# tmoroney/whisper-diarize-rs

Measured on AMD Instinct MI355X. Metric: audio-sec/wall-sec (xRT), large-v3 + DTW + diarize, 1/2/4/8 MI355X, higher is better.
Workload: dtype f16 (f32 accumulate)

## Files before the change

include/wdr.h:

```cpp
#ifndef WDR_H
#define WDR_H

#include <stddef.h>
#include <stdint.h>

#ifdef __cplusplus
extern "C" {
#endif

#define WDR_ABI_VERSION 6

typedef struct wdr_engine wdr_engine;
typedef struct wdr_context wdr_context;

typedef struct {
  const char* cache_dir;
  int8_t enable_dtw;
  int8_t enable_flash_attn;
  int8_t use_gpu;
  int8_t has_gpu_device;
  int32_t gpu_device;
  const char* vad_model_path;
  const char* diarize_segment_model_path;
  const char* diarize_embedding_model_path;
// ... 74 lines not shown
  double start, end;
  const int16_t* samples; size_t n_samples;
} wdr_speech_segment;

typedef struct {
  void* user;
  void (*progress)(void* user, int32_t pct, int32_t type , const char* label);
  void (*new_segment)(void* user, const wdr_segment* seg);
  int (*is_cancelled)(void* user);
} wdr_callbacks;

typedef struct {
  double mel, encode, decode, dtw, vad, total;
  int64_t windows, decode_steps, prefills;
  double lang, prompt_gpu, embed;
  int64_t chains, batch_launches, batch_rows, fixup_segments, replay_segments;
  double spec_s, fixup_s;
  double batch_step_s;
  int64_t early_fixup_segments;
  int64_t batch_prefill_rows, batch_dtw_rows, batch_prefills, batch_dtws, batch_mixed;
  int64_t batch_xattn_groups, batch_xattn_tiles;
  int64_t dtwq_passes, dtwq_rows, dtwq_jobs;
  int64_t lang_passes, lang_rows;
} wdr_stage_times;

const char* wdr_last_error(void);
int wdr_abi_version(void);
int wdr_device_count(void);
void wdr_shutdown(void);

int wdr_engine_new(const wdr_engine_config* cfg, wdr_engine** out);
void wdr_engine_free(wdr_engine* e);
int wdr_engine_set_synthetic(wdr_engine* e, const wdr_synthetic* syn);
int wdr_engine_set_audio_convert(wdr_engine* e, int8_t on);
int wdr_engine_set_channel_split(wdr_engine* e, int8_t on);
int wdr_transcribe_audio(wdr_engine* e, const char* audio_path, const wdr_transcribe_options* opts,
                         const wdr_formatting_overrides* fmt, const wdr_callbacks* cb, wdr_segment_list** out);

int wdr_read_wav(const char* path, int16_t** samples, size_t* n);
int wdr_audio_info(const char* path, int32_t* info, uint64_t* n_frames);
int wdr_read_audio(const char* path, int8_t has_gpu_device, int32_t gpu_device, int16_t** samples, size_t* n);
int wdr_read_audio_channels(const char* path, int8_t has_gpu_device, int32_t gpu_device,
                            int16_t** samples, size_t* n_per_channel, int32_t* channels);
int wdr_dbg_model_file(int32_t kind, const char* path, char** names_out, float** data_out, size_t* n_values);
int wdr_process_segments(const wdr_segment* segs, size_t n_segs, const char* lang, const wdr_formatting_overrides* ov,
                         int8_t has_mask, const double* vad_mask, size_t n_mask, wdr_segment_list** out);
void wdr_free(void* p);
int wdr_vad_merge(const double* starts_cs, const double* ends_cs, size_t n_segs, const int16_t* samples,
                  size_t n_samples, double* mask_out , size_t* n_mask,
                  double* merged_out , int64_t* merged_idx ,
                  size_t* n_merged);
typedef struct wdr_vad wdr_vad;
int wdr_vad_create(const char* model_path, int8_t has_gpu_device, int32_t gpu_device, wdr_vad** out);
void wdr_vad_free(wdr_vad* v);
int wdr_vad_probs(wdr_vad* v, const int16_t* samples, size_t n, float* probs_out, double* us_per_step);
int wdr_vad_stats(wdr_vad* v, double* us_per_chunk);
int wdr_vad_segments_from_probs(const float* probs, size_t n_probs, float* cs_out, size_t* n_out);
int wdr_vad_get_segments(wdr_vad* v, const int16_t* samples, size_t n, double** mask_out, size_t* n_mask,
                         wdr_speech_segment** segs_out, size_t* n_segs);

typedef struct wdr_diarizer wdr_diarizer;
int wdr_diarizer_create(const char* segment_model_path, const char* embedding_model_path, int8_t has_gpu_device,
                        int32_t gpu_device, wdr_diarizer** out);
void wdr_diarizer_free(wdr_diarizer* d);
int wdr_diarize_frame_classes(wdr_diarizer* d, const int16_t* samples, size_t n, int32_t* cls_out, float* logprobs_out);
int wdr_diarize_get_segments(wdr_diarizer* d, const int16_t* samples, size_t n, wdr_speech_segment** segs_out,
                             size_t* n_segs);
int wdr_diarize_segments_from_classes(const int32_t* cls, size_t n_windows, const int16_t* samples, size_t n,
                                      wdr_speech_segment** segs_out, size_t* n_segs);
int wdr_diarize_fbank(wdr_diarizer* d, const int16_t* samples, size_t n, float* feats_out, size_t* n_frames);
int wdr_diarize_embedding(wdr_diarizer* d, const int16_t* samples, size_t n, float* emb_out, int8_t* ok);
int wdr_diarize_embedding_batch(wdr_diarizer* d, const int16_t* const* samples, const size_t* n, int32_t B,
                                float* emb_out, int8_t* ok);
int wdr_diarize_stats(wdr_diarizer* d, double* seg_ms, double* emb_ms);
typedef struct wdr_speakers wdr_speakers;
int wdr_speakers_new(int8_t has_max_speakers, uint64_t max_speakers, wdr_speakers** out);
void wdr_speakers_free(wdr_speakers* m);
int wdr_speakers_assign(wdr_speakers* m, const float* emb, int32_t dim, float threshold, char* id_out, size_t cap);

int wdr_context_create(const char* model_path, const char* model_name, int8_t has_gpu_device, int32_t gpu_device,
                       int8_t use_gpu, int8_t enable_dtw, int8_t enable_flash_attn, int8_t has_num_samples,
                       uint64_t num_samples, const wdr_synthetic* syn, wdr_context** out);
void wdr_context_free(wdr_context* c);
int wdr_ggml_info(const char* path, int32_t* hparams, int64_t* n_tensors, int64_t* n_vocab_tokens);
int wdr_ggml_tensor_types(const char* path, int64_t* counts );
int wdr_ggml_tensor_f16(const char* path, const char* name, uint16_t** out, size_t* n);
int wdr_run_pipeline(wdr_context* c, const wdr_speech_segment* segs, size_t n_segs, const wdr_transcribe_options* opts,
                     const wdr_diarize_options* diarize, const wdr_synthetic* syn, const wdr_callbacks* cb,
                     wdr_segment_list** out);
int wdr_run_pipeline_raw(wdr_context* c, const wdr_speech_segment* segs, size_t n_segs,
                         const wdr_transcribe_options* opts, const wdr_synthetic* syn, wdr_segment_list** out);
int wdr_run_pipeline_block(wdr_context* c, const wdr_speech_segment* segs, size_t n_segs,
                           const wdr_transcribe_options* opts, const wdr_synthetic* syn, const char* rng_in,
                           int8_t* sampled_out, char** rng_out, wdr_segment_list** out);
void wdr_segment_list_free(wdr_segment_list* l);
int wdr_context_set_chains(wdr_context* c, int32_t n);
int wdr_context_devices(const wdr_context* c, int32_t* n, int32_t* device_ids, int32_t cap);
int wdr_context_set_encoder_fp8(wdr_context* c, int8_t on);
int wdr_dbg_set_early_fixup(wdr_context* c, int32_t mode);
int wdr_dbg_set_gemm32(int32_t mfma);
int wdr_context_stage_times(wdr_context* c, wdr_stage_times* out);
int wdr_context_hparams(wdr_context* c, int32_t* out );

int wdr_prof_set(int32_t cls);
int wdr_prof_set_mask(int32_t mask);
int wdr_prof_read_class(int32_t cls, double* total_ms, int64_t* launches, double* algo_bytes, double* algo_flops);
int wdr_prof_read_clock(int32_t cls, double* total_ms, int64_t* launches, double* algo_bytes, double* algo_flops);
int wdr_prof_read(double* total_ms, int64_t* launches, double* algo_bytes, double* algo_flops);

typedef struct {
  int32_t id, tid;
  float p, plog, pt, ptsum;
  int64_t t0, t1, t_dtw;
} wdr_token;
typedef struct {
  int64_t t0, t1;
  const char* text;
  const wdr_token* tokens; size_t n_tokens;
} wdr_result_seg;
int wdr_state_full(wdr_context* c, const float* samples, size_t n, const wdr_transcribe_options* opts,
                   const wdr_synthetic* syn, const char* initial_prompt, wdr_result_seg** segs, size_t* n_segs,
                   int32_t* lang_id);
void wdr_result_free(wdr_result_seg* segs, size_t n);

int wdr_dbg_log_mel(wdr_context* c, const float* x, size_t n, int32_t seek, float* window_out );
int wdr_dbg_energy(const float* x, size_t n, float* out);
int wdr_dbg_dequant(int32_t type, const uint8_t* blocks, size_t n_blocks, uint16_t* out_f16, double* ms);
int wdr_dbg_audio_convert(const uint8_t* raw, uint64_t n_frames, int32_t fmt, int32_t channels, int32_t rate,
                          uint64_t chunk_frames, int32_t host, int16_t** out, size_t* n_out, double* ms);
int wdr_dbg_audio_split(const uint8_t* raw, uint64_t n_frames, int32_t fmt, int32_t channels, int32_t rate,
                        uint64_t chunk_frames, int32_t host, int16_t** out, size_t* n_per_channel, double* ms);
int wdr_dbg_resample_table(int32_t rate, int32_t* L, int32_t* M, int32_t* T, float** tab);
int wdr_dbg_mfma_scale(const uint8_t* a, const uint8_t* b, const int32_t* sa, const int32_t* sb, float* out);
int wdr_dbg_encode(wdr_context* c, const float* mel_window , float* enc_out );
int wdr_dbg_cross_kv(wdr_context* c, float* out);
int wdr_dbg_decode(wdr_context* c, const int32_t* tokens, size_t n, float* logits_out );
int wdr_dbg_step(wdr_context* c, const int32_t* tokens, size_t n, float* logits_out );
int wdr_dbg_logits(wdr_context* c, const float* logits, int32_t R, const int32_t* ctl, const float* temperature,
                   float max_initial_ts, int32_t suppress_blank, int32_t* ids_out, float* f_out);
int wdr_dbg_batch_step(wdr_context* c, const int32_t* tokens, size_t n, int32_t rows, int32_t iters,
                       double* ms_per_step);
int wdr_dbg_capture(wdr_context* c, const int32_t* tokens, size_t n, float* cap_out );
int wdr_dbg_dtw(const float* cap, int32_t n_heads, int32_t n_tok, int32_t n_audio, int32_t sot_len, int32_t seek,
                float* x_out , int32_t* times_out, int32_t* n_times);
int wdr_dbg_discrete(const float* w, size_t n, uint32_t seed, int32_t n_draws, int32_t* out);
int wdr_dbg_dtw_dp(const float* x, int32_t rows, int32_t cols, int32_t seek, int32_t* times_out, int32_t* n_times);
int wdr_dbg_proj_fp8(const uint16_t* a_f16, const uint16_t* w_f16, const float* bias, int32_t M, int32_t N, int32_t K,
                     int32_t epi, float* out, uint8_t* a8_out, uint8_t* a_scale_out, uint8_t* w8_out,
                     uint8_t* w_scale_out);
int wdr_dbg_proj(const uint16_t* a_f16, const uint16_t* w_f16, const float* bias, int32_t M, int32_t N, int32_t K,
                 int32_t epi, float* out );
#define WDR_DBG_PROJ_ROWS 0x200
#define WDR_DBG_PROJ_GEMM1 0x800
int wdr_dbg_proj_ln(const float* x, const float* gamma, const float* beta, const uint16_t* w_f16, const float* bias,
                    int32_t M, int32_t N, int32_t K, int32_t epi, int32_t fused, float* out);
int wdr_dbg_attn(const uint16_t* q, const uint16_t* k, const uint16_t* v, int32_t Tq, int32_t Tk, int32_t n_head,
                 int32_t causal, float* out );
int wdr_dbg_xattn(const uint16_t* q, const uint16_t* kv, const int32_t* row_slot, const int32_t* grp, int32_t R,
                  int32_t S, int32_t H, int32_t iters, float* out);

int wdr_dbg_self_attn(const uint16_t* q, const uint16_t* kc, const uint16_t* vc, int32_t n_seq, int32_t T,
                      const int32_t* row_seq, const int32_t* row_pos, int32_t R, int32_t H, float* out);
int wdr_dbg_proj_qkv(const uint16_t* a_f16, const uint16_t* w_f16, const float* bias, int32_t M, int32_t d, int32_t K,
                     const int32_t* row_seq, const int32_t* row_pos, int32_t n_seq, int32_t T, uint16_t* kc_io,
                     uint16_t* vc_io, float* q_out);
int wdr_dbg_logits_topk(wdr_context* c, const float* logits, int32_t R, const int32_t* ctl, const float* temperature,
                        float max_initial_ts, int32_t suppress_blank, int32_t K, int32_t* ids_out, float* f_out);
int wdr_dbg_logits_probs(wdr_context* c, const float* logits, int32_t R, const int32_t* ctl, const float* temperature,
                         float max_initial_ts, int32_t suppress_blank, float* probs_out, float* logprobs_out);
int wdr_dbg_kv_rows(wdr_context* c, int32_t seq, int32_t n_rows, int32_t write, uint16_t* k, uint16_t* v);
int wdr_dbg_kv_reorder(wdr_context* c, const int32_t* src, const int32_t* dst, int32_t n, int32_t n_rows);

#ifdef __cplusplus
}
#endif
#endif
```

whisper-diarize-rs_amd/csrc/common.h:

```cpp
#pragma once

#include <hip/hip_runtime.h>
#include <hip/hip_fp16.h>

#include <cstdint>
#include <cstdio>
#include <stdexcept>
#include <string>

namespace wdr {

struct HipError : std::runtime_error {
  using std::runtime_error::runtime_error;
};

#define WDR_HIP(call)                                                                       \
  do {                                                                                      \
    hipError_t e_ = (call);                                                                 \
    if (e_ != hipSuccess)                                                                   \
      throw ::wdr::HipError(std::string("HIP error ") + hipGetErrorString(e_) + " at " +    \
                            __FILE__ + ":" + std::to_string(__LINE__) + " (" #call ")");    \
  } while (0)

#define WDR_CHECK(cond, msg)                                                                \
  do {                                                                                      \
    if (!(cond)) throw std::runtime_error(std::string(msg));                                \
  } while (0)

typedef _Float16 f16;
typedef _Float16 f16x8 __attribute__((ext_vector_type(8)));
typedef _Float16 f16x4 __attribute__((ext_vector_type(4)));
typedef float f32x16 __attribute__((ext_vector_type(16)));
typedef float f32x4 __attribute__((ext_vector_type(4)));

enum Epi : int {
  EPI_F16 = 0,
  EPI_F16_GELU = 1,
  EPI_F32_RESID = 2,
  EPI_F32 = 3,
  EPI_F32_GELU_POS = 4,
  EPI_QKV_CACHE = 5,
  EPI_XKV = 6,
  EPI_F8_GELU = 7
};

constexpr int XKV_T = 1500;
constexpr long long XKV_HS = (long long)XKV_T * 64;
__host__ __device__ inline long long xkv_k_off(int l, int H) { return (long long)(2 * l) * H * XKV_HS; }
__host__ __device__ inline long long xkv_v_off(int l, int H) { return (long long)(2 * l + 1) * H * XKV_HS; }

__host__ __device__ inline int cdiv(int a, int b) { return (a + b - 1) / b; }

__device__ __forceinline__ float gelu_tanh(float x) {
#pragma clang fp contract(off)
  const float c2 = 2.0f * 0.7978845608028654f;
  const float u2 = c2 * __builtin_fmaf(0.044715f * x, x * x, x);
  float g = x * __builtin_amdgcn_rcpf(1.0f + __builtin_amdgcn_exp2f(u2 * -1.4426950408889634f));
  asm("" : "+v"(g));
  return g;
}

__device__ __forceinline__ float wave_sum(float v) {
  for (int o = 32; o > 0; o >>= 1) v += __shfl_xor(v, o, 64);
  return v;
}
__device__ __forceinline__ float wave_max(float v) {
  for (int o = 32; o > 0; o >>= 1) v = fmaxf(v, __shfl_xor(v, o, 64));
  return v;
}
__device__ __forceinline__ void lds_barrier() { asm volatile("s_waitcnt lgkmcnt(0)\n\ts_barrier" ::: "memory"); }

__device__ __forceinline__ double wave_sum_d(double v) {
  for (int o = 32; o > 0; o >>= 1) v += __shfl_xor(v, o, 64);
  return v;
}

struct ProjArgs {
  const f16* A; int lda;
  const f16* B; int ldb;
  const float* bias;
  void* out; int ldo;
  const float* pos; int pos_rows;
  int M, N, K;
  int epi;
  const float* ln_x = nullptr; int ldln = 0; const float* ln_g = nullptr; const float* ln_b = nullptr;
  f16* kc = nullptr; f16* vc = nullptr; long long seq_stride = 0; const int* row_seq = nullptr;
  const int* row_pos = nullptr; int d = 0;
  unsigned long long* ts = nullptr;
  const uint8_t* A8 = nullptr; const uint8_t* B8 = nullptr;
  const uint32_t* a_sc = nullptr; const uint32_t* b_sc = nullptr; int ld_asc = 0, ld_bsc = 0;
  uint32_t* o_sc = nullptr; int ld_osc = 0;
  int tile_gm = 0;
  int gemm_ref = 0;
  int rows_mma = 0;
  const int* row_map = nullptr;
};

constexpr int PROF_CLK_LANES = 128;
struct ProfClock {
  unsigned long long* ts;
  __device__ __forceinline__ explicit ProfClock(unsigned long long* t) : ts(t) {
    if (ts && threadIdx.x == 0) atomicMin(ts + lane_of_block(), (unsigned long long)wall_clock64());
  }
  __device__ __forceinline__ ~ProfClock() {
    if (ts && threadIdx.x == ((blockDim.x - 1) & ~63u)) atomicMax(ts + PROF_CLK_LANES + lane_of_block(), (unsigned long long)wall_clock64());
  }
  __device__ __forceinline__ static int lane_of_block() {
    return (int)((blockIdx.x + blockIdx.y * 7u + blockIdx.z * 13u) % PROF_CLK_LANES);
  }
};
unsigned long long* prof_slot();
template <typename A>
inline unsigned long long* prof_attach(A&) { return nullptr; }
inline unsigned long long* prof_attach(ProjArgs& a) { return a.ts = prof_slot(); }
void launch_proj(const ProjArgs& a, hipStream_t s);
void gemm_knobs_reload();
void launch_proj_fp8(const ProjArgs& a, hipStream_t s);
void launch_quant_f8(const f16* x, int ldx, int rows, int K, uint8_t* y, int ldy, uint32_t* sc, int ld_sc,
                     hipStream_t s);
void launch_probe_mfma_scale(const void* a, const void* b, const int* sa, const int* sb, float* out, hipStream_t s);
void launch_layernorm_f8(const float* x, int ldx, const float* g, const float* b, uint8_t* y, int ldy, uint32_t* sc,
                         int ld_sc, int rows, int d, hipStream_t s);

}
```

whisper-diarize-rs_amd/csrc/engine.cpp:

```cpp
#include <algorithm>
#include <atomic>
#include <chrono>
#include <cmath>
#include <cstdio>
#include <cstdlib>
#include <cstring>
#include <fstream>
#include <map>
#include <memory>
#include <random>
#include <string>
#include <sys/stat.h>
#include <dirent.h>
#include <condition_variable>
#include <exception>
#include <mutex>
#include <set>
#include <pthread.h>
#include <thread>
#include <vector>

#include "../../include/wdr.h"
#include "audio_file.h"
#include "audio_gpu.h"
// ... 2233 lines not shown

int wdr_dbg_decode(wdr_context* c, const int32_t* tokens, size_t n, float* logits_out) {
  WDR_GUARD({
    WDR_USE(ctx, c);
    c->st->decode_logits(tokens, (int)n, logits_out);
    return 0;
  })
}

int wdr_dbg_step(wdr_context* c, const int32_t* tokens, size_t n, float* logits_out) {
  WDR_GUARD({
    WDR_USE(ctx, c);
    c->st->dbg_step(tokens, (int)n, logits_out);
    return 0;
  })
}

int wdr_dbg_logits(wdr_context* c, const float* logits, int32_t R, const int32_t* ctl, const float* temperature,
                   float max_initial_ts, int32_t suppress_blank, int32_t* ids_out, float* f_out) {
  WDR_GUARD({
    WDR_USE(ctx, c);
    WDR_CHECK(R >= 1 && R <= 8, "dbg_logits: 1..8 rows");
    std::vector<LogitsCtl> lc(R);
    for (int r = 0; r < R; ++r) {
      const int32_t* q = ctl + 7 * r;
      lc[r] = LogitsCtl{q[0], q[1], q[2], q[3], q[4], q[5], q[6], temperature[r]};
    }
    std::vector<TokenData> out(R);
    std::vector<float> nosp(R);
    c->st->dbg_logits(logits, R, lc.data(), max_initial_ts, suppress_blank != 0, out.data(), nosp.data());
    for (int r = 0; r < R; ++r) {
      ids_out[2 * r] = out[r].id;
      ids_out[2 * r + 1] = out[r].tid;
      float* f = f_out + 5 * r;
      f[0] = out[r].p;
      f[1] = out[r].plog;
      f[2] = out[r].pt;
      f[3] = out[r].ptsum;
      f[4] = nosp[r];
    }
    return 0;
  })
}

int wdr_dbg_batch_step(wdr_context* c, const int32_t* tokens, size_t n, int32_t rows, int32_t iters,
                       double* ms_per_step) {
  WDR_GUARD({
    WDR_USE(ctx, c);
    *ms_per_step = c->st->dbg_batch_step(tokens, (int)n, rows, iters);
    return 0;
  })
}

int wdr_dbg_capture(wdr_context* c, const int32_t* tokens, size_t n, float* cap_out) {
  WDR_GUARD({
    WDR_USE(ctx, c);
    if (c->ctx->aheads.empty()) return fail("context created without DTW");
    c->st->dtw_capture(tokens, (int)n, cap_out);
    return 0;
  })
}

int wdr_dbg_dtw(const float* cap, int32_t A, int32_t N, int32_t M, int32_t sot_len, int32_t seek, float* x_out,
                int32_t* times_out, int32_t* n_times) {
  WDR_GUARD({
    DevMem dcap((size_t)A * N * 1500 * 4), dn((size_t)A * N * M * 4), dx((size_t)N * M * 4), dt((N + 8) * 4);
    WDR_HIP(hipMemcpy(dcap.p, cap, dcap.bytes, hipMemcpyHostToDevice));
    launch_dtw(dcap.as<float>(), A, N, 1500, M, sot_len, seek, dn.as<float>(), dx.as<float>(), dt.as<int>(),
               dt.as<int>() + N + 4, nullptr);
    WDR_HIP(hipDeviceSynchronize());
    const int rows = N - sot_len - 1;
    WDR_HIP(hipMemcpy(x_out, dx.p, (size_t)rows * M * 4, hipMemcpyDeviceToHost));
    std::vector<int> t(N + 8);
    WDR_HIP(hipMemcpy(t.data(), dt.p, t.size() * 4, hipMemcpyDeviceToHost));
    *n_times = t[N + 4];
    for (int i = 0; i < *n_times; ++i) times_out[i] = t[i];
    return 0;
  })
}

int wdr_dbg_dtw_dp(const float* x, int32_t rows, int32_t cols, int32_t seek, int32_t* times_out, int32_t* n_times) {
  WDR_GUARD({
    DevMem dx((size_t)rows * cols * 4), dt((rows + 8) * 4);
    WDR_HIP(hipMemcpy(dx.p, x, dx.bytes, hipMemcpyHostToDevice));
    launch_dtw_dp_only(dx.as<float>(), rows, cols, seek, dt.as<int>(), dt.as<int>() + rows + 4, nullptr);
    std::vector<int> t(rows + 8);
    WDR_HIP(hipMemcpy(t.data(), dt.p, t.size() * 4, hipMemcpyDeviceToHost));
    *n_times = t[rows + 4];
    for (int i = 0; i < *n_times; ++i) times_out[i] = t[i];
    return 0;
  })
}

int wdr_dbg_proj_fp8(const uint16_t* a16, const uint16_t* w16, const float* bias, int32_t M, int32_t N, int32_t K,
                     int32_t epi, float* out, uint8_t* a8_out, uint8_t* a_sc_out, uint8_t* w8_out, uint8_t* w_sc_out) {
  WDR_GUARD({
    WDR_CHECK(M > 64 && N % 256 == 0 && K % 128 == 0, "dbg fp8 projection: M > 64, N % 256, K % 128");
    const int mp = (M + 255) / 256 * 256;
    DevMem da((size_t)M * K * 2), dw((size_t)N * K * 2), db(bias ? (size_t)N * 4 : 0), dout((size_t)M * N * 4);
    DevMem a8((size_t)M * K), w8((size_t)N * K), as((size_t)K / 128 * mp * 4), ws((size_t)K / 128 * N * 4);
    DevMem osc((size_t)N / 128 * mp * 4);
    WDR_HIP(hipMemcpy(da.p, a16, da.bytes, hipMemcpyHostToDevice));
    WDR_HIP(hipMemcpy(dw.p, w16, dw.bytes, hipMemcpyHostToDevice));
    if (bias) WDR_HIP(hipMemcpy(db.p, bias, db.bytes, hipMemcpyHostToDevice));
    launch_quant_f8(da.as<f16>(), K, M, K, a8.as<uint8_t>(), K, as.as<uint32_t>(), mp, nullptr);
    launch_quant_f8(dw.as<f16>(), K, N, K, w8.as<uint8_t>(), K, ws.as<uint32_t>(), N, nullptr);
    const bool f16out = epi == EPI_F16 || epi == EPI_F16_GELU;
    if (!f16out && epi != EPI_F8_GELU) WDR_HIP(hipMemcpy(dout.p, out, dout.bytes, hipMemcpyHostToDevice));
    ProjArgs p{nullptr, K, nullptr, K, bias ? db.as<float>() : nullptr, dout.p, N, nullptr, 0, M, N, K, epi};
    p.A8 = a8.as<uint8_t>();
    p.a_sc = as.as<uint32_t>();
    p.ld_asc = mp;
    p.B8 = w8.as<uint8_t>();
    p.b_sc = ws.as<uint32_t>();
    p.ld_bsc = N;
    p.o_sc = osc.as<uint32_t>();
    p.ld_osc = mp;
    launch_proj_fp8(p, nullptr);
    WDR_HIP(hipDeviceSynchronize());
    auto unscale = [](const DevMem& d, int rows, int ld, int K, uint8_t* dst) {
      std::vector<uint32_t> h(d.bytes / 4);
      WDR_HIP(hipMemcpy(h.data(), d.p, d.bytes, hipMemcpyDeviceToHost));
      for (int r = 0; r < rows; ++r)
        for (int b = 0; b < K / 32; ++b) dst[(size_t)r * (K / 32) + b] = (uint8_t)(h[(size_t)(b / 4) * ld + r] >> (8 * (b % 4)));
    };
    if (epi == EPI_F8_GELU) {
      std::vector<uint8_t> q((size_t)M * N), sc((size_t)M * (N / 32));
      WDR_HIP(hipMemcpy(q.data(), dout.p, q.size(), hipMemcpyDeviceToHost));
      unscale(osc, M, mp, N, sc.data());
      for (int r = 0; r < M; ++r)
        for (int c = 0; c < N; ++c) {
          const uint8_t v = q[(size_t)r * N + c];
          const int e = (v >> 3) & 15, mt = v & 7;
          float x = e ? std::ldexp(1.0f + mt / 8.0f, e - 7) : std::ldexp(mt / 8.0f, -6);
          if ((v & 0x7f) == 0x7f) x = NAN;
          x = (v & 0x80) ? -x : x;
          out[(size_t)r * N + c] = std::ldexp(x, (int)sc[(size_t)r * (N / 32) + c / 32] - 127);
        }
    } else if (f16out) {
      std::vector<f16> h((size_t)M * N);
      WDR_HIP(hipMemcpy(h.data(), dout.p, h.size() * 2, hipMemcpyDeviceToHost));
      for (size_t i = 0; i < h.size(); ++i) out[i] = (float)h[i];
    } else {
      WDR_HIP(hipMemcpy(out, dout.p, dout.bytes, hipMemcpyDeviceToHost));
    }
    if (a8_out) WDR_HIP(hipMemcpy(a8_out, a8.p, a8.bytes, hipMemcpyDeviceToHost));
    if (a_sc_out) unscale(as, M, mp, K, a_sc_out);
    if (w8_out) WDR_HIP(hipMemcpy(w8_out, w8.p, w8.bytes, hipMemcpyDeviceToHost));
    if (w_sc_out) unscale(ws, N, N, K, w_sc_out);
    return 0;
  })
}

int wdr_dbg_proj(const uint16_t* a16, const uint16_t* w16, const float* bias, int32_t M, int32_t N, int32_t K,
                 int32_t epi, float* out) {
  WDR_GUARD({
    DevMem da((size_t)M * K * 2), dw((size_t)N * K * 2), db(bias ? (size_t)N * 4 : 0), dout((size_t)M * N * 4);
    WDR_HIP(hipMemcpy(da.p, a16, da.bytes, hipMemcpyHostToDevice));
    WDR_HIP(hipMemcpy(dw.p, w16, dw.bytes, hipMemcpyHostToDevice));
    if (bias) WDR_HIP(hipMemcpy(db.p, bias, db.bytes, hipMemcpyHostToDevice));
    if (epi & 0x100) return fail("WDR_DBG_PROJ_STEP: the decode-step GEMV schedule was removed (the row kernel serves every row count)");
    const bool rows = (epi & 0x200) != 0;
    if (epi & 0x400) return fail("WDR_DBG_PROJ_SPLIT: the split-K residual projections were removed (k_skinny runs them whole)");
    const bool gemm_ref = (epi & 0x800) != 0;
    epi &= 0xff;
    const bool f16out = epi == EPI_F16 || epi == EPI_F16_GELU;
    std::vector<f16> h16;
    if (!f16out) WDR_HIP(hipMemcpy(dout.p, out, dout.bytes, hipMemcpyHostToDevice));
    ProjArgs a{da.as<f16>(), K, dw.as<f16>(), K, bias ? db.as<float>() : nullptr, dout.p, N, nullptr, 0, M, N, K, epi};
    a.rows_mma = rows ? 1 : 0;
    a.gemm_ref = gemm_ref ? 1 : 0;
    launch_proj(a, nullptr);
    WDR_HIP(hipDeviceSynchronize());
    if (f16out) {
      h16.resize((size_t)M * N);
      WDR_HIP(hipMemcpy(h16.data(), dout.p, h16.size() * 2, hipMemcpyDeviceToHost));
      for (size_t i = 0; i < h16.size(); ++i) out[i] = (float)h16[i];
    } else {
      WDR_HIP(hipMemcpy(out, dout.p, dout.bytes, hipMemcpyDeviceToHost));
    }
    return 0;
  })
}

int wdr_dbg_proj_ln(const float* x, const float* gamma, const float* beta, const uint16_t* w16, const float* bias,
                    int32_t M, int32_t N, int32_t K, int32_t epi, int32_t fused, float* out) {
  WDR_GUARD({
    if (M < 1 || N < 1 || K < 128 || K > 1280 || K % 128) return fail("dbg_proj_ln: M >= 1, K % 128 == 0, K <= 1280");
    if (epi != EPI_F16 && epi != EPI_F16_GELU && epi != EPI_F32) return fail("dbg_proj_ln: epi 0, 1 or 3");
    DevMem dx((size_t)M * K * 4), dg((size_t)K * 4), dbt((size_t)K * 4), dw((size_t)N * K * 2),
        db(bias ? (size_t)N * 4 : 0), dh((size_t)M * K * 2), dout((size_t)M * N * 4);
    WDR_HIP(hipMemcpy(dx.p, x, dx.bytes, hipMemcpyHostToDevice));
    WDR_HIP(hipMemcpy(dg.p, gamma, dg.bytes, hipMemcpyHostToDevice));
    WDR_HIP(hipMemcpy(dbt.p, beta, dbt.bytes, hipMemcpyHostToDevice));
    WDR_HIP(hipMemcpy(dw.p, w16, dw.bytes, hipMemcpyHostToDevice));
    if (bias) WDR_HIP(hipMemcpy(db.p, bias, db.bytes, hipMemcpyHostToDevice));
    ProjArgs a{nullptr, K, dw.as<f16>(), K, bias ? db.as<float>() : nullptr, dout.p, N, nullptr, 0, M, N, K, epi};
    a.rows_mma = 1;
    if (fused) {
      a.ln_x = dx.as<float>();
      a.ldln = K;
      a.ln_g = dg.as<float>();
      a.ln_b = dbt.as<float>();
    } else {
      launch_layernorm(dx.as<float>(), K, dg.as<float>(), dbt.as<float>(), dh.as<f16>(), K, M, K, nullptr);
      a.A = dh.as<f16>();
    }
    launch_proj(a, nullptr);
    WDR_HIP(hipDeviceSynchronize());
    if (epi == EPI_F32) {
      WDR_HIP(hipMemcpy(out, dout.p, dout.bytes, hipMemcpyDeviceToHost));
    } else {
      std::vector<f16> h((size_t)M * N);
      WDR_HIP(hipMemcpy(h.data(), dout.p, h.size() * 2, hipMemcpyDeviceToHost));
      for (size_t i = 0; i < h.size(); ++i) out[i] = (float)h[i];
    }
    return 0;
  })
}

int wdr_dbg_attn(const uint16_t* q, const uint16_t* k, const uint16_t* v, int32_t Tq, int32_t Tk, int32_t H,
                 int32_t causal, float* out) {
  WDR_GUARD({
    const int d = H * 64;
    DevMem dq((size_t)Tq * d * 2), dk((size_t)Tk * d * 2), dv((size_t)Tk * d * 2), dout((size_t)Tq * d * 2);
    WDR_HIP(hipMemcpy(dq.p, q, dq.bytes, hipMemcpyHostToDevice));
    WDR_HIP(hipMemcpy(dk.p, k, dk.bytes, hipMemcpyHostToDevice));
    WDR_HIP(hipMemcpy(dv.p, v, dv.bytes, hipMemcpyHostToDevice));
    FlashArgs fa{dq.as<f16>(), d, 0, dk.as<f16>(), d, 0, dv.as<f16>(), d, 0, dout.as<f16>(), d, 0, nullptr, Tq, Tk, H,
                 causal, 0.125f};
    DevMem po, pml;
    if (!causal && Tq <= 256 && Tk >= 512) {
      fa.nsplit = 12;
      po = DevMem((size_t)12 * Tq * H * 64 * 4);
      pml = DevMem((size_t)12 * H * Tq * 8);
      fa.part_o = po.as<float>();
      fa.part_ml = pml.as<float2>();
    }
    launch_flash_attn(fa, 1, nullptr);
    std::vector<f16> h((size_t)Tq * d);
    WDR_HIP(hipMemcpy(h.data(), dout.p, h.size() * 2, hipMemcpyDeviceToHost));
    for (size_t i = 0; i < h.size(); ++i) out[i] = (float)h[i];
    return 0;
  })
}

int wdr_dbg_xattn(const uint16_t* q, const uint16_t* kv, const int32_t* row_slot, const int32_t* grp, int32_t R,
                  int32_t S, int32_t H, int32_t iters, float* out) {
  WDR_GUARD({
    WDR_CHECK(R >= 1 && R <= 1024 && S >= 1 && H >= 1 && H <= 32 && iters >= 1, "dbg xattn: bad shape");
    const int d = H * 64, T = 1500;
    DevMem dq((size_t)R * d * 2), dkv((size_t)S * T * 2 * d * 2), dout((size_t)R * d * 2);
    DevMem po((size_t)24 * R * H * 64 * 4), pml((size_t)24 * R * H * 8);
    DevMem drk(R * sizeof(void*)), dg(R * 4), dl(R * 4);
    WDR_HIP(hipMemcpy(dq.p, q, dq.bytes, hipMemcpyHostToDevice));
    WDR_HIP(hipMemcpy(dkv.p, kv, dkv.bytes, hipMemcpyHostToDevice));
    XAttnArgs xa{dq.as<f16>(), d, dkv.as<f16>(), dkv.as<f16>() + d, 2 * d, T, R, H, 0.125f, po.as<float>(),
                 pml.as<float2>(), dout.as<f16>(), d};
    if (row_slot) {
      std::vector<const f16*> rk(R);
      for (int r = 0; r < R; ++r) {
        WDR_CHECK(row_slot[r] >= 0 && row_slot[r] < S, "dbg xattn: slot out of range");
        rk[r] = dkv.as<f16>() + (size_t)row_slot[r] * T * 2 * d;
      }
      WDR_HIP(hipMemcpy(drk.p, rk.data(), R * sizeof(void*), hipMemcpyHostToDevice));
      xa.row_k = drk.as<const f16*>();
      xa.v_off = d;
      bool big = false;
      for (int r = 0; grp && r < R; ++r) big = big || grp[r] > XATTN_GRP_MAX;
      if (grp && big) {
        std::vector<int> g(R, 0), lead;
        std::vector<int4> tiles;
        for (int r = 0; r < R; ++r) {
          if (grp[r] == 0) continue;
          WDR_CHECK(r + grp[r] <= R, "dbg xattn: bad group");
          if (grp[r] <= XATTN_GRP_MAX) {
            g[r] = grp[r];
            lead.push_back(r);
          } else {
            for (int t = 0; t < grp[r]; t += 128) tiles.push_back(make_int4(r + t, std::min(128, grp[r] - t), 1 << 30, 0));
          }
        }
        WDR_HIP(hipMemcpy(dg.p, g.data(), R * 4, hipMemcpyHostToDevice));
        if (!lead.empty()) WDR_HIP(hipMemcpy(dl.p, lead.data(), lead.size() * 4, hipMemcpyHostToDevice));
        DevMem dt(std::max<size_t>(16, tiles.size() * 16));
        if (!tiles.empty()) WDR_HIP(hipMemcpy(dt.p, tiles.data(), tiles.size() * 16, hipMemcpyHostToDevice));
        xa.grp = dg.as<int>();
        xa.lead = dl.as<int>();
        xa.n_vgrp = (int)lead.size();
        xa.vgrp_max = 1;
        for (int r : lead) xa.vgrp_max = std::max(xa.vgrp_max, g[r]);
        xa.tiles = dt.as<int4>();
        xa.n_tiles = (int)tiles.size();
        for (int i = 0; i < iters; ++i) launch_xattn_rows(xa, nullptr);
        WDR_HIP(hipDeviceSynchronize());
        std::vector<f16> h((size_t)R * d);
        WDR_HIP(hipMemcpy(h.data(), dout.p, h.size() * 2, hipMemcpyDeviceToHost));
        for (size_t i = 0; i < h.size(); ++i) out[i] = (float)h[i];
        return 0;
      }
      if (grp) {
        int ng = 0;
        for (int r = 0; r < R; ++r) {
          WDR_CHECK(grp[r] >= 0 && grp[r] <= XATTN_GRP_MAX && r + grp[r] <= R, "dbg xattn: bad group");
          ng += grp[r] > 0;
        }
        WDR_HIP(hipMemcpy(dg.p, grp, R * 4, hipMemcpyHostToDevice));
        xa.grp = dg.as<int>();
        xa.n_grp = ng;
        std::vector<int> lead;
        for (int r = 0; r < R; ++r)
          if (grp[r] > 0) lead.push_back(r);
        WDR_HIP(hipMemcpy(dl.p, lead.data(), lead.size() * 4, hipMemcpyHostToDevice));
        xa.lead = dl.as<int>();
      }
    }
    for (int i = 0; i < iters; ++i) launch_xattn(xa, nullptr);
    WDR_HIP(hipDeviceSynchronize());
    std::vector<f16> h((size_t)R * d);
    WDR_HIP(hipMemcpy(h.data(), dout.p, h.size() * 2, hipMemcpyDeviceToHost));
    for (size_t i = 0; i < h.size(); ++i) out[i] = (float)h[i];
    return 0;
  })
}

static void check_rows(const int32_t* row_seq, const int32_t* row_pos, int R, int n_seq, int T, const char* what) {
  for (int r = 0; r < R; ++r) {
    WDR_CHECK(row_seq[r] >= 0 && row_seq[r] < n_seq, std::string(what) + ": row_seq out of range");
    WDR_CHECK(row_pos[r] >= 0 && row_pos[r] < std::min(T, 448), std::string(what) + ": row_pos out of range");
  }
}

int wdr_dbg_self_attn(const uint16_t* q, const uint16_t* kc, const uint16_t* vc, int32_t n_seq, int32_t T,
                      const int32_t* row_seq, const int32_t* row_pos, int32_t R, int32_t H, float* out) {
  WDR_GUARD({
    WDR_CHECK(q && kc && vc && row_seq && row_pos && out, "dbg self-attn: null argument");
    WDR_CHECK(R >= 1 && R <= 4096 && H >= 1 && H <= 32 && n_seq >= 1 && n_seq <= 64 && T >= 1 && T <= 4096,
              "dbg self-attn: bad shape");
    check_rows(row_seq, row_pos, R, n_seq, T, "dbg self-attn");
    const int d = H * 64;
    const size_t cache = (size_t)n_seq * T * d * 2;
    DevMem dq((size_t)R * d * 2), dk(cache), dv(cache), dout((size_t)R * d * 2), ds(R * 4), dp(R * 4);
    WDR_HIP(hipMemcpy(dq.p, q, dq.bytes, hipMemcpyHostToDevice));
    WDR_HIP(hipMemcpy(dk.p, kc, cache, hipMemcpyHostToDevice));
    WDR_HIP(hipMemcpy(dv.p, vc, cache, hipMemcpyHostToDevice));
    WDR_HIP(hipMemcpy(ds.p, row_seq, R * 4, hipMemcpyHostToDevice));
    WDR_HIP(hipMemcpy(dp.p, row_pos, R * 4, hipMemcpyHostToDevice));
    DecSelfArgs sa{dq.as<f16>(), d, dk.as<f16>(), dv.as<f16>(), (long long)T * d, d, ds.as<int>(), dp.as<int>(),
                   dout.as<f16>(), d, 0.125f};
    launch_dec_self_attn(sa, R, H, nullptr);
    WDR_HIP(hipDeviceSynchronize());
    std::vector<f16> h((size_t)R * d);
    WDR_HIP(hipMemcpy(h.data(), dout.p, h.size() * 2, hipMemcpyDeviceToHost));
    for (size_t i = 0; i < h.size(); ++i) out[i] = (float)h[i];
    return 0;
  })
}

int wdr_dbg_proj_qkv(const uint16_t* a16, const uint16_t* w16, const float* bias, int32_t M, int32_t d, int32_t K,
                     const int32_t* row_seq, const int32_t* row_pos, int32_t n_seq, int32_t T, uint16_t* kc_io,
                     uint16_t* vc_io, float* q_out) {
  WDR_GUARD({
    WDR_CHECK(a16 && w16 && row_seq && row_pos && kc_io && vc_io && q_out, "dbg qkv projection: null argument");
    WDR_CHECK(M >= 1 && M <= 4096 && d >= 64 && d <= 2048 && d % 64 == 0 && d % 8 == 0 && K >= 32 && K <= 8192 &&
                  K % 32 == 0 && n_seq >= 1 && n_seq <= 64 && T >= 1 && T <= 4096,
              "dbg qkv projection: bad shape (d = 64 H, K % 32)");
    check_rows(row_seq, row_pos, M, n_seq, T, "dbg qkv projection");
    std::set<long long> seen;
    for (int r = 0; r < M; ++r)
      WDR_CHECK(seen.insert((long long)row_seq[r] * T + row_pos[r]).second, "dbg qkv projection: a cache row named twice");
    const int N = 3 * d;
    const size_t cache = (size_t)n_seq * T * d * 2;
    DevMem da((size_t)M * K * 2), dw((size_t)N * K * 2), db(bias ? (size_t)N * 4 : 0), dq((size_t)M * d * 2), dk(cache),
        dv(cache), ds(M * 4), dp(M * 4);
    WDR_HIP(hipMemcpy(da.p, a16, da.bytes, hipMemcpyHostToDevice));
    WDR_HIP(hipMemcpy(dw.p, w16, dw.bytes, hipMemcpyHostToDevice));
    if (bias) WDR_HIP(hipMemcpy(db.p, bias, db.bytes, hipMemcpyHostToDevice));
    WDR_HIP(hipMemcpy(dk.p, kc_io, cache, hipMemcpyHostToDevice));
    WDR_HIP(hipMemcpy(dv.p, vc_io, cache, hipMemcpyHostToDevice));
    WDR_HIP(hipMemcpy(ds.p, row_seq, M * 4, hipMemcpyHostToDevice));
    WDR_HIP(hipMemcpy(dp.p, row_pos, M * 4, hipMemcpyHostToDevice));
    ProjArgs a{da.as<f16>(), K, dw.as<f16>(), K, bias ? db.as<float>() : nullptr, dq.p, d, nullptr, 0, M, N, K,
               EPI_QKV_CACHE};
    a.rows_mma = 1;
    a.kc = dk.as<f16>();
    a.vc = dv.as<f16>();
    a.seq_stride = (long long)T * d;
    a.row_seq = ds.as<int>();
    a.row_pos = dp.as<int>();
    a.d = d;
    launch_proj(a, nullptr);
    WDR_HIP(hipDeviceSynchronize());
    std::vector<f16> h((size_t)M * d);
    WDR_HIP(hipMemcpy(h.data(), dq.p, h.size() * 2, hipMemcpyDeviceToHost));
    for (size_t i = 0; i < h.size(); ++i) q_out[i] = (float)h[i];
    WDR_HIP(hipMemcpy(kc_io, dk.p, cache, hipMemcpyDeviceToHost));
    WDR_HIP(hipMemcpy(vc_io, dv.p, cache, hipMemcpyDeviceToHost));
    return 0;
  })
}

static void dbg_ctls(const int32_t* ctl, const float* temperature, int R, std::vector<LogitsCtl>& lc) {
  lc.resize(R);
  for (int r = 0; r < R; ++r) {
    const int32_t* q = ctl + 7 * r;
    lc[r] = LogitsCtl{q[0], q[1], q[2], q[3], q[4], q[5], q[6], temperature[r]};
  }
}

int wdr_dbg_logits_topk(wdr_context* c, const float* logits, int32_t R, const int32_t* ctl, const float* temperature,
                        float max_initial_ts, int32_t suppress_blank, int32_t K, int32_t* ids_out, float* f_out) {
  WDR_GUARD({
    WDR_USE(ctx, c);
    WDR_CHECK(logits && ctl && temperature && ids_out && f_out, "dbg_logits_topk: null argument");
    WDR_CHECK(R >= 1 && R <= 8, "dbg_logits_topk: 1..8 rows");
    WDR_CHECK(K >= 1 && K <= BEAM_KMAX, "dbg_logits_topk: K out of range");
    std::vector<LogitsCtl> lc;
    dbg_ctls(ctl, temperature, R, lc);
    std::vector<BeamCand> bc((size_t)R * K);
    c->st->dbg_logits_topk(logits, R, lc.data(), max_initial_ts, suppress_blank != 0, K, bc.data());
    for (int i = 0; i < R * K; ++i) {
      ids_out[i] = bc[i].id;
      f_out[2 * i] = bc[i].p;
      f_out[2 * i + 1] = bc[i].plog;
    }
    return 0;
  })
}

int wdr_dbg_logits_probs(wdr_context* c, const float* logits, int32_t R, const int32_t* ctl, const float* temperature,
                         float max_initial_ts, int32_t suppress_blank, float* probs_out, float* logprobs_out) {
  WDR_GUARD({
    WDR_USE(ctx, c);
    WDR_CHECK(logits && ctl && temperature && probs_out && logprobs_out, "dbg_logits_probs: null argument");
    WDR_CHECK(R >= 1 && R <= 8, "dbg_logits_probs: 1..8 rows");
    std::vector<LogitsCtl> lc;
    dbg_ctls(ctl, temperature, R, lc);
    c->st->dbg_logits_probs(logits, R, lc.data(), max_initial_ts, suppress_blank != 0, probs_out, logprobs_out);
    return 0;
  })
}

int wdr_dbg_kv_rows(wdr_context* c, int32_t seq, int32_t n_rows, int32_t write, uint16_t* k, uint16_t* v) {
  WDR_GUARD({
    WDR_USE(ctx, c);
    WDR_CHECK(k && v, "dbg_kv_rows: null argument");
    c->st->dbg_kv_rows(seq, n_rows, write != 0, k, v);
    return 0;
  })
}

int wdr_dbg_kv_reorder(wdr_context* c, const int32_t* src, const int32_t* dst, int32_t n, int32_t n_rows) {
  WDR_GUARD({
    WDR_USE(ctx, c);
    WDR_CHECK(src && dst, "dbg_kv_reorder: null argument");
    c->st->dbg_kv_reorder(src, dst, n, n_rows);
    return 0;
  })
}

}
```

whisper-diarize-rs_amd/csrc/kernels/gemm.hip:

```cpp
#include "../common.h"
#include "../prof.h"

#include <algorithm>
#include <cstdlib>

namespace wdr {

typedef _Float16 f16x2 __attribute__((ext_vector_type(2)));

constexpr int GB_M = 128, GB_N = 128, GB_K = 32;
constexpr int GLDS = GB_K + 8;

template <int EPI>
__device__ __forceinline__ void epi_store(const ProjArgs& a, int row, int col, float v) {
  if (row >= a.M || col >= a.N) return;
  if (a.bias) v += a.bias[col];
  if constexpr (EPI == EPI_F16) {
    ((f16*)a.out)[(size_t)row * a.ldo + col] = (f16)v;
  } else if constexpr (EPI == EPI_F16_GELU) {
    ((f16*)a.out)[(size_t)row * a.ldo + col] = (f16)gelu_tanh(v);
  } else if constexpr (EPI == EPI_F32_RESID) {
    float* o = (float*)a.out + (size_t)row * a.ldo + col;
    *o = *o + v;
  } else if constexpr (EPI == EPI_F32) {
// ... 1111 lines not shown
      static bool attrn = [] {
        WDR_HIP(hipFuncSetAttribute((const void*)k_gemm8n<EPI>, hipFuncAttributeMaxDynamicSharedMemorySize, (int)G8N_LDS));
        return true;
      }();
      (void)attrn;
      const int ntn = (a.N / 128) * cdiv(a.M, G3_M);
      wdr_launch(PROF_GEMM, bytes, flops, k_gemm8n<EPI>, dim3(ntn), dim3(512), G8N_LDS, s, g);
      return;
    }
  }
  const int ntiles = (a.N / G3_N) * cdiv(a.M, G3_M);
  wdr_launch(PROF_GEMM, bytes, flops, k_gemm8<EPI>, dim3(ntiles), dim3(512), G8_LDS, s, g);
}

void launch_proj_fp8(const ProjArgs& a, hipStream_t s) {
  WDR_CHECK(a.A8 && a.B8 && a.a_sc && a.b_sc, "fp8 projection: operands / scales missing");
  WDR_CHECK(a.M > 64 && a.N % 128 == 0 && (a.epi != EPI_F8_GELU || a.N % G3_N == 0) && a.K % G8_BK == 0 &&
                a.lda % 16 == 0 && a.ldb % 16 == 0,
            "fp8 projection: M > 64, N % 128 == 0 (N % 256 for the GELU -> fp8 epilogue), K % 128 == 0, "
            "lda / ldb % 16 required");
  WDR_CHECK(a.ld_asc >= cdiv(a.M, G3_M) * G3_M && a.ld_bsc >= a.N && a.ld_asc % 4 == 0 && a.ld_bsc % 4 == 0,
            "fp8 projection: scale images need the rows rounded up to 256");
  WDR_CHECK(a.epi != EPI_F8_GELU || (a.o_sc && a.ld_osc >= cdiv(a.M, G3_M) * G3_M && a.ldo % 16 == 0),
            "fp8 projection: GELU -> fp8 epilogue needs an output scale image");
  switch (a.epi) {
    case EPI_F16: launch_epi8<EPI_F16>(a, s); break;
    case EPI_F16_GELU: launch_epi8<EPI_F16_GELU>(a, s); break;
    case EPI_F32_RESID: launch_epi8<EPI_F32_RESID>(a, s); break;
    case EPI_F32: launch_epi8<EPI_F32>(a, s); break;
    case EPI_F8_GELU: launch_epi8<EPI_F8_GELU>(a, s); break;
    default: throw std::runtime_error("fp8 projection: unsupported epilogue");
  }
  WDR_HIP(hipGetLastError());
}

__global__ __launch_bounds__(256) void k_quant_f8(const f16* x, int ldx, int rows, int K, uint8_t* y, int ldy,
                                                  uint32_t* sc, int ld_sc) {
  const int row = blockIdx.x * 4 + (threadIdx.x >> 6), lane = threadIdx.x & 63;
  if (row >= rows) return;
  const f16* xr = x + (size_t)row * ldx;
  for (int c0 = 0; c0 < K; c0 += 512) {
    const int c = c0 + lane * 8;
    const bool ok = c < K;
    f16x8 v = ok ? *(const f16x8*)(xr + c) : f16x8{};
    float am = 0.f;
#pragma unroll
    for (int e = 0; e < 8; ++e) am = fmaxf(am, fabsf((float)v[e]));
    am = fmaxf(am, __shfl_xor(am, 1, 64));
    am = fmaxf(am, __shfl_xor(am, 2, 64));
    const int e = f8_block_exp(am);
    const float inv = f8_pow2(-e);
    const uint32_t lo = f8_pack4((float)v[0] * inv, (float)v[1] * inv, (float)v[2] * inv, (float)v[3] * inv);
    const uint32_t hi = f8_pack4((float)v[4] * inv, (float)v[5] * inv, (float)v[6] * inv, (float)v[7] * inv);
    if (ok) *(uint2*)(y + (size_t)row * ldy + c) = make_uint2(lo, hi);
    const int b = e + 127, base = lane & ~15;
    const uint32_t w = (uint32_t)__shfl(b, base, 64) | (uint32_t)__shfl(b, base + 4, 64) << 8 |
                       (uint32_t)__shfl(b, base + 8, 64) << 16 | (uint32_t)__shfl(b, base + 12, 64) << 24;
    if ((lane & 15) == 0 && ok) sc[(size_t)(c >> 7) * ld_sc + row] = w;
  }
}

__global__ __launch_bounds__(64) void k_probe_mfma_scale(const i32x8* a, const i32x8* b, const int* sa, const int* sb,
                                                          f32x4* out) {
  const int l = threadIdx.x;
  out[l] = __builtin_amdgcn_mfma_scale_f32_16x16x128_f8f6f4(a[l], b[l], f32x4{0.f, 0.f, 0.f, 0.f}, 0, 0, 0, sa[l], 0,
                                                             sb[l]);
}
void launch_probe_mfma_scale(const void* a, const void* b, const int* sa, const int* sb, float* out, hipStream_t s) {
  WDR_KLAUNCH(k_probe_mfma_scale, dim3(1), dim3(64), 0, s, (const i32x8*)a, (const i32x8*)b, sa, sb, (f32x4*)out);
  WDR_HIP(hipGetLastError());
}

void launch_quant_f8(const f16* x, int ldx, int rows, int K, uint8_t* y, int ldy, uint32_t* sc, int ld_sc,
                     hipStream_t s) {
  WDR_CHECK(rows >= 1 && K % 128 == 0 && ldx % 8 == 0 && ldy % 16 == 0 && ld_sc >= rows,
            "fp8 quantisation: K % 128, ldx % 8, ldy % 16, scale rows");
  WDR_KLAUNCH(k_quant_f8, dim3(cdiv(rows, 4)), dim3(256), 0, s, x, ldx, rows, K, y, ldy, sc, ld_sc);
  WDR_HIP(hipGetLastError());
}

__global__ __launch_bounds__(256) void k_layernorm_f8(const float* x, int ldx, const float* g, const float* b,
                                                      uint8_t* y, int ldy, uint32_t* sc, int ld_sc, int rows, int d) {
  const int row = blockIdx.x * 4 + (threadIdx.x >> 6);
  const int lane = threadIdx.x & 63;
  if (row >= rows) return;
  const float* xr = x + (long long)row * ldx;
  float v[5][4];
  float s = 0.f;
#pragma unroll
  for (int j = 0; j < 5; ++j) {
    const int c = lane * 4 + j * 256;
    const bool ok = c < d;
    const int cc = ok ? c : 0;
    const float4 q = *(const float4*)(xr + cc);
    v[j][0] = ok ? q.x : 0.f; v[j][1] = ok ? q.y : 0.f; v[j][2] = ok ? q.z : 0.f; v[j][3] = ok ? q.w : 0.f;
    s += (v[j][0] + v[j][1]) + (v[j][2] + v[j][3]);
  }
  s = wave_sum(s);
  const float mean = s / d;
  float s2 = 0.f;
#pragma unroll
  for (int j = 0; j < 5; ++j)
    if (lane * 4 + j * 256 < d)
#pragma unroll
      for (int e = 0; e < 4; ++e) {
        const float t = v[j][e] - mean;
        s2 += t * t;
      }
  s2 = wave_sum(s2);
  const float scale = 1.0f / sqrtf(s2 / d + 1e-5f);
#pragma unroll
  for (int j = 0; j < 5; ++j) {
    const int c = lane * 4 + j * 256;
    if (j * 256 >= d) break;
    const bool ok = c < d;
    const int cc = ok ? c : 0;
    const float4 g4 = *(const float4*)(g + cc);
    const float4 b4 = *(const float4*)(b + cc);
    const float gg[4] = {g4.x, g4.y, g4.z, g4.w}, bb[4] = {b4.x, b4.y, b4.z, b4.w};
    float o[4], am = 0.f;
#pragma unroll
    for (int e = 0; e < 4; ++e) {
      o[e] = ok ? (v[j][e] - mean) * scale * gg[e] + bb[e] : 0.f;
      am = fmaxf(am, fabsf(o[e]));
    }
    am = fmaxf(am, __shfl_xor(am, 1, 64));
    am = fmaxf(am, __shfl_xor(am, 2, 64));
    am = fmaxf(am, __shfl_xor(am, 4, 64));
    const int e = f8_block_exp(am);
    const float inv = f8_pow2(-e);
    if (ok) *(uint32_t*)(y + (size_t)row * ldy + c) = f8_pack4(o[0] * inv, o[1] * inv, o[2] * inv, o[3] * inv);
    const int bb8 = e + 127, base = lane & 32;
    const uint32_t w = (uint32_t)__shfl(bb8, base, 64) | (uint32_t)__shfl(bb8, base + 8, 64) << 8 |
                       (uint32_t)__shfl(bb8, base + 16, 64) << 16 | (uint32_t)__shfl(bb8, base + 24, 64) << 24;
    if ((lane & 31) == 0 && ok) sc[(size_t)(c >> 7) * ld_sc + row] = w;
  }
}

void launch_layernorm_f8(const float* x, int ldx, const float* g, const float* b, uint8_t* y, int ldy, uint32_t* sc,
                         int ld_sc, int rows, int d, hipStream_t s) {
  WDR_CHECK(d % 128 == 0 && d <= 1280 && ldx % 4 == 0 && ldy % 16 == 0 && ld_sc >= rows,
            "fp8 layernorm: d % 128, d <= 1280");
  WDR_KLAUNCH(k_layernorm_f8, dim3(cdiv(rows, 4)), dim3(256), 0, s, x, ldx, g, b, y, ldy, sc, ld_sc, rows, d);
  WDR_HIP(hipGetLastError());
}

template <int EPI, int MT, int NT, int W>
constexpr uint32_t skinny_red_bytes() { return (uint32_t)W * MT * NT * 4 * 64 * 4; }
template <int EPI, int MT, int NT, int W>
static uint32_t skinny_ln_lds(int K) {
  return std::max((uint32_t)16 * MT * K * 2, skinny_red_bytes<EPI, MT, NT, W>());
}

template <int EPI, int MT, int NT, int W = 4, bool LN = false, int UU = 0>
__global__ __launch_bounds__(W * 64) void k_skinny(ProjArgs a) {
  ProfClock prof_clock_(a.ts);
  __shared__ float red_s[LN ? 1 : W * MT * NT * 4 * 64];
  extern __shared__ __attribute__((aligned(16))) f16 xln[];
  float* red = LN ? (float*)xln : red_s;
  const int lane = threadIdx.x & 63, wid = threadIdx.x >> 6;
  const int n0 = blockIdx.x * 16 * NT;
  const int m0 = blockIdx.y * 16 * MT;
  const int fr = lane & 15, fk = 8 * (lane >> 4);
  f32x4 acc[MT][NT];
#pragma unroll
  for (int i = 0; i < MT; ++i)
#pragma unroll
    for (int j = 0; j < NT; ++j) acc[i][j] = (f32x4){0.f, 0.f, 0.f, 0.f};
  const int lds_ld = a.K;
  if constexpr (LN) {
    const int d = a.K;
    const int live = min(16 * MT, a.M - m0);
    for (int rr = wid; rr < live; rr += W) {
      int row = m0 + rr;
      if (a.row_map) row = a.row_map[row];
      const float* xr = a.ln_x + (long long)row * a.ldln;
      float v[5][4];
      float sm = 0.f;
#pragma unroll
      for (int j = 0; j < 5; ++j) {
        const int c = lane * 4 + j * 256;
        const bool ok = c < d;
        const int cc = ok ? c : 0;
        const float4 q = *(const float4*)(xr + cc);
        v[j][0] = ok ? q.x : 0.f; v[j][1] = ok ? q.y : 0.f; v[j][2] = ok ? q.z : 0.f; v[j][3] = ok ? q.w : 0.f;
        sm += (v[j][0] + v[j][1]) + (v[j][2] + v[j][3]);
      }
      sm = wave_sum(sm);
      const float mean = sm / d;
      float s2 = 0.f;
#pragma unroll
      for (int j = 0; j < 5; ++j)
        if (lane * 4 + j * 256 < d)
#pragma unroll
          for (int e = 0; e < 4; ++e) {
            const float t = v[j][e] - mean;
            s2 += t * t;
          }
      s2 = wave_sum(s2);
      const float scale = 1.0f / sqrtf(s2 / d + 1e-5f);
#pragma unroll
      for (int j = 0; j < 5; ++j) {
        const int c = lane * 4 + j * 256;
        if (c >= d) continue;
        const float4 g4 = *(const float4*)(a.ln_g + c);
        const float4 b4 = *(const float4*)(a.ln_b + c);
        const float gg[4] = {g4.x, g4.y, g4.z, g4.w}, bb[4] = {b4.x, b4.y, b4.z, b4.w};
        f16x4 o;
#pragma unroll
        for (int e = 0; e < 4; ++e) o[e] = (f16)((v[j][e] - mean) * scale * gg[e] + bb[e]);
        *(f16x4*)(xln + rr * lds_ld + ((((c >> 3) ^ (rr & 15))) << 3) + (c & 7)) = o;
      }
    }
    __syncthreads();
  }
  const f16* arow[MT];
#pragma unroll
  for (int i = 0; i < MT; ++i) {
    int m = m0 + i * 16 + fr;
    m = m < a.M ? m : a.M - 1;
    if (!LN && a.row_map) m = a.row_map[m];
    arow[i] = LN ? xln + (i * 16 + fr) * lds_ld : a.A + (size_t)m * a.lda + fk;
  }
  const f16* brow[NT];
#pragma unroll
  for (int j = 0; j < NT; ++j) {
    int n = n0 + j * 16 + fr;
    n = n < a.N ? n : a.N - 1;
    brow[j] = a.B + (size_t)n * a.ldb + fk;
  }
  constexpr int U = UU > 0 ? UU : (MT + NT) <= 3 ? 8 : 4;
  for (int k0 = wid * 32; k0 < a.K; k0 += 32 * W * U) {
    f16x8 bf[U][NT], af[U][MT];
#pragma unroll
    for (int u = 0; u < U; ++u) {
      const int k = k0 + u * 32 * W;
      const bool ok = k < a.K;
      const int kk = ok ? k : 0;
#pragma unroll
      for (int j = 0; j < NT; ++j) {
        const f16x8 t = *(const f16x8*)(brow[j] + kk);
        bf[u][j] = ok ? t : (f16x8){};
      }
#pragma unroll
      for (int i = 0; i < MT; ++i) {
        const f16x8 t = LN ? *(const f16x8*)(arow[i] + ((((kk >> 3) | (lane >> 4)) ^ fr) << 3))
                           : *(const f16x8*)(arow[i] + kk);
        af[u][i] = ok ? t : (f16x8){};
      }
    }
#pragma unroll
    for (int u = 0; u < U; ++u)
#pragma unroll
      for (int i = 0; i < MT; ++i)
#pragma unroll
        for (int j = 0; j < NT; ++j)
          acc[i][j] = __builtin_amdgcn_mfma_f32_16x16x32_f16(af[u][i], bf[u][j], acc[i][j], 0, 0, 0);
  }
  if constexpr (LN) __syncthreads();
#pragma unroll
  for (int i = 0; i < MT; ++i)
#pragma unroll
    for (int j = 0; j < NT; ++j)
#pragma unroll
      for (int r = 0; r < 4; ++r) red[(((wid * MT + i) * NT + j) * 4 + r) * 64 + lane] = acc[i][j][r];
  __syncthreads();
  for (int e = threadIdx.x; e < MT * NT * 4 * 64; e += W * 64) {
    const int l = e & 63, r = (e >> 6) & 3, j = (e >> 8) % NT, i = (e >> 8) / NT;
    float v = 0.f;
#pragma unroll
    for (int w = 0; w < W; ++w) v += red[(((w * MT + i) * NT + j) * 4 + r) * 64 + l];
    const int row = m0 + i * 16 + (l >> 4) * 4 + r, col = n0 + j * 16 + (l & 15);
    epi_store<EPI>(a, row, col, v);
  }
}



struct GemmKnobs {
  bool gemm1, gemm3, gemm5, gemm5w;
  int gemm4, tile_gm, cus;
};
static int env_int(const char* name, int def) {
  const char* e = getenv(name);
  return e ? atoi(e) : def;
}
static GemmKnobs read_knobs() {
  GemmKnobs k;
  k.gemm1 = env_int("WDR_GEMM1", 0) != 0;
  k.gemm3 = env_int("WDR_GEMM3", 1) != 0 && !k.gemm1;
  k.gemm4 = env_int("WDR_GEMM4", -1);
  k.tile_gm = env_int("WDR_GEMM4_GM", 4);
  k.gemm5 = env_int("WDR_GEMM5", 0) != 0;
  k.gemm5w = env_int("WDR_GEMM5_WIDE", 1) != 0;
  k.cus = env_int("WDR_GEMM_CUS", 0) / 8 * 8;
  return k;
}
static GemmKnobs& knobs() {
  static GemmKnobs k = read_knobs();
  return k;
}
void gemm_knobs_reload() { knobs() = read_knobs(); }

template <int EPI>
static void launch_epi(const ProjArgs& a, hipStream_t s) {
  const int ob = (EPI == EPI_F32_RESID || EPI == EPI_F32 || EPI == EPI_F32_GELU_POS) ? 4 : 2;
  const double bytes = (double)a.N * a.K * 2 + (double)a.M * a.K * 2 + (double)a.M * a.N * ob;
  const double flops = 2.0 * a.M * a.N * a.K;
  WDR_CHECK(a.M > 64, "encoder GEMM: more than 64 rows (fewer go to the row kernel)");
  const GemmKnobs& kn = knobs();
  const bool ref = kn.gemm1 || a.gemm_ref;
  const bool vec4 = a.ldo % 4 == 0 && (a.epi != EPI_QKV_CACHE || a.d % 4 == 0);
  const bool wide5 = kn.gemm5w && a.N >= 4096 && a.N < 16384 && a.M >= 4096;
  if (a.N % 128 == 0 && a.K % G3_BK == 0 && a.M >= 4096 && !ref && vec4 && kn.gemm4 != 0 &&
      (wide5 || (a.N < 2048 && kn.gemm5 && (a.N / G3_N) * cdiv(a.M, G3_M) < 192))) {
    static bool attr5 = [] {
      WDR_HIP(hipFuncSetAttribute((const void*)k_gemm5<EPI>, hipFuncAttributeMaxDynamicSharedMemorySize, (int)G5_LDS));
      return true;
    }();
    (void)attr5;
    ProjArgs g = a;
    g.tile_gm = kn.tile_gm;
    const int ntiles5 = (a.N / 128) * cdiv(a.M, G3_M);
    dim3 grid(kn.cus > 0 && kn.cus < ntiles5 ? kn.cus : ntiles5);
    wdr_launch(PROF_GEMM, bytes, flops, k_gemm5<EPI>, grid, dim3(512), G5_LDS, s, g);
  } else if (a.N % G3_N == 0 && a.K % G3_BK == 0 && !ref && vec4 &&
             (kn.gemm4 == 1 ||
              (kn.gemm4 != 0 && (a.M >= 4096 || a.N >= 16384 || (a.N >= 4096 && a.M > 1024) ||
                                 (a.N >= 3072 && a.M >= 2560))))) {
    static bool attr4 = [] {
      WDR_HIP(hipFuncSetAttribute((const void*)k_gemm4<EPI>, hipFuncAttributeMaxDynamicSharedMemorySize, (int)G4_LDS));
      return true;
    }();
    (void)attr4;
    const int ntiles = (a.N / G3_N) * cdiv(a.M, G3_M);
    dim3 grid(kn.cus > 0 && kn.cus < ntiles ? kn.cus : ntiles);
    ProjArgs g = a;
    g.tile_gm = kn.tile_gm;
    wdr_launch(PROF_GEMM, bytes, flops, k_gemm4<EPI>, grid, dim3(512), G4_LDS, s, g);
  } else if ((a.N >= 5120 || a.M >= 9000) && a.M > 2048 && a.N % G3_N == 0 && a.K % G3_BK == 0 && kn.gemm3 && !ref) {
    static bool attr = [] {
      WDR_HIP(hipFuncSetAttribute((const void*)k_gemm3<EPI>, hipFuncAttributeMaxDynamicSharedMemorySize, (int)G3_LDS));
      return true;
    }();
    (void)attr;
    dim3 grid((a.N / G3_N) * cdiv(a.M, G3_M));
    wdr_launch(PROF_GEMM, bytes, flops, k_gemm3<EPI>, grid, dim3(512), G3_LDS, s, a);
  } else if (a.K % G2_BK == 0 && a.N <= 4096 && !ref && vec4) {
    dim3 grid((a.N / GB_N) * cdiv(a.M, GB_M));
    wdr_launch(PROF_GEMM, bytes, flops, k_gemm2<EPI>, grid, dim3(256), 0, s, a);
  } else {
    dim3 grid(a.N / GB_N, cdiv(a.M, GB_M));
    wdr_launch(PROF_GEMM, bytes, flops, k_gemm<EPI>, grid, dim3(256), 0, s, a);
  }
}

static bool rows_pair_tiles() {
  static const bool v = env_int("WDR_ROWS_PAIR", 1) != 0;
  return v;
}
static int rows_mt_max() {
  static const int v = std::max(2, std::min(5, env_int("WDR_ROWS_MT", 2)));
  return v;
}

template <int EPI>
static void launch_rows_epi(const ProjArgs& a, hipStream_t s) {
  const double bytes = (double)a.N * a.K * 2;
  const double flops = 2.0 * a.M * a.N * a.K;
  const int mt = cdiv(a.M, 16);
  const bool ln = a.ln_x != nullptr;
  const bool wide = a.N >= 4096;
  const int prof = PROF_GEMV;
  if (!wide) {
    if (a.K > 2048) {
      WDR_CHECK(!ln, "row projection: LN prologue needs K <= 1280");
      if (mt >= 4 && rows_pair_tiles()) {
        const int m2 = std::min(mt, rows_mt_max());
        const dim3 g2(cdiv(a.N, 16), cdiv(mt, m2));
        if (m2 >= 4) wdr_launch(prof, bytes, flops, k_skinny<EPI, 4, 1, 16, false, 2>, g2, dim3(1024), 0, s, a);
        else if (m2 == 3) wdr_launch(prof, bytes, flops, k_skinny<EPI, 3, 1, 16, false, 5>, g2, dim3(1024), 0, s, a);
        else wdr_launch(prof, bytes, flops, k_skinny<EPI, 2, 1, 16, false, 5>, g2, dim3(1024), 0, s, a);
        return;
      }
      wdr_launch(prof, bytes, flops, k_skinny<EPI, 1, 1, 16, false, 12>, dim3(cdiv(a.N, 16), mt), dim3(1024), 0, s, a);
      return;
    }
    if (!ln && mt > 2 && rows_pair_tiles()) {
      const int m2 = std::min(mt, rows_mt_max());
      const dim3 g2(cdiv(a.N, 16), cdiv(mt, m2));
      if (m2 >= 5) wdr_launch(prof, bytes, flops, k_skinny<EPI, 5, 1, 8>, g2, dim3(512), 0, s, a);
      else if (m2 == 4) wdr_launch(prof, bytes, flops, k_skinny<EPI, 4, 1, 8>, g2, dim3(512), 0, s, a);
      else if (m2 == 3) wdr_launch(prof, bytes, flops, k_skinny<EPI, 3, 1, 8>, g2, dim3(512), 0, s, a);
      else wdr_launch(prof, bytes, flops, k_skinny<EPI, 2, 1, 8>, g2, dim3(512), 0, s, a);
      return;
    }
    dim3 grid(cdiv(a.N, 16), mt), blk(512);
    if (ln) wdr_launch(prof, bytes, flops, k_skinny<EPI, 1, 1, 8, true>, grid, blk, skinny_ln_lds<EPI, 1, 1, 8>(a.K), s, a);
    else wdr_launch(prof, bytes, flops, k_skinny<EPI, 1, 1, 8>, grid, blk, 0, s, a);
    return;
  }
  const int mtw = std::min(mt, ln ? 2 : 4);
  dim3 grid(cdiv(a.N, 32), cdiv(mt, mtw)), blk(512);
#define WDR_RW(MTV)                                                                                        \
  if (ln) wdr_launch(prof, bytes, flops, k_skinny<EPI, MTV, 2, 8, true>, grid, blk, skinny_ln_lds<EPI, MTV, 2, 8>(a.K), s, a); \
  else wdr_launch(prof, bytes, flops, k_skinny<EPI, MTV, 2, 8>, grid, blk, 0, s, a);
  if (mtw == 1) { WDR_RW(1) }
  else if (mtw == 2) { WDR_RW(2) }
  else if (mtw == 3) { WDR_RW(3) }
  else { WDR_RW(4) }
#undef WDR_RW
}

static void launch_rows(const ProjArgs& a, hipStream_t s) {
  WDR_CHECK(a.K % 32 == 0 && a.lda % 8 == 0 && a.ldb % 8 == 0, "row projection: K % 32, lda / ldb % 8");
  WDR_CHECK(!a.ln_x || (a.K <= 1280 && a.K % 128 == 0), "row projection LN prologue: K <= 1280, K % 128 == 0");
  WDR_CHECK(a.epi != EPI_QKV_CACHE || (a.kc && a.vc && a.row_seq && a.row_pos && a.d > 0), "qkv-cache epilogue args");
  switch (a.epi) {
    case EPI_F16: launch_rows_epi<EPI_F16>(a, s); break;
    case EPI_F16_GELU: launch_rows_epi<EPI_F16_GELU>(a, s); break;
    case EPI_F32_RESID: launch_rows_epi<EPI_F32_RESID>(a, s); break;
    case EPI_F32: launch_rows_epi<EPI_F32>(a, s); break;
    case EPI_QKV_CACHE: launch_rows_epi<EPI_QKV_CACHE>(a, s); break;
    default: throw std::runtime_error("row projection: bad epilogue");
  }
  WDR_HIP(hipGetLastError());
}

void launch_proj(const ProjArgs& a, hipStream_t s) {
  WDR_CHECK(a.M > 0 && a.K > 0 && a.N > 0, "projection: empty shape");
  if (a.rows_mma || a.M <= 64) {
    launch_rows(a, s);
    return;
  }
  WDR_CHECK(a.K % 8 == 0 && a.lda % 8 == 0 && a.ldb % 8 == 0, "projection: K/lda/ldb must be multiples of 8");
  WDR_CHECK(a.N % GB_N == 0, "gemm: N must be a multiple of 128");
  WDR_CHECK(a.K % GB_K == 0, "gemm: K must be a multiple of 32");
  WDR_CHECK(a.epi != EPI_QKV_CACHE || (a.kc && a.vc && a.row_seq && a.row_pos && a.d > 0), "qkv-cache epilogue args");
  switch (a.epi) {
    case EPI_F16: launch_epi<EPI_F16>(a, s); break;
    case EPI_F16_GELU: launch_epi<EPI_F16_GELU>(a, s); break;
    case EPI_F32_RESID: launch_epi<EPI_F32_RESID>(a, s); break;
    case EPI_F32: launch_epi<EPI_F32>(a, s); break;
    case EPI_F32_GELU_POS: launch_epi<EPI_F32_GELU_POS>(a, s); break;
    case EPI_QKV_CACHE: launch_epi<EPI_QKV_CACHE>(a, s); break;
    case EPI_XKV:
      WDR_CHECK(a.M > 64 && a.seq_stride > 0, "cross-K/V epilogue: encoder GEMM rows and a slot stride");
      launch_epi<EPI_XKV>(a, s);
      break;
    default: throw std::runtime_error("projection: bad epilogue");
  }
  WDR_HIP(hipGetLastError());
}

}
```

whisper-diarize-rs_amd/csrc/rows.cpp:

```cpp
#include "rows.h"
#include "prof.h"

#include <algorithm>
#include <cstdlib>
#include <cstring>

namespace wdr {

namespace {
constexpr int kTileRows = 128;
constexpr int kNoEnd = 1 << 30;
size_t up16(size_t x) { return (x + 15) & ~size_t(15); }
}

RowBatch::RowBatch(int cr, int cl, int cc) : cap_rows(cr), cap_logits(cl), cap_caps(cc) {
  std::lock_guard<std::recursive_mutex> g(hip_alloc_mutex());
  bytes_ = up16((size_t)cr * 4) * 5 + up16((size_t)cr * 4) + up16((size_t)cl * 4) + 2 * up16((size_t)cc * 4) +
           up16((size_t)(cr / 8 + 2 + cr / kTileRows + 2) * 16) + up16((size_t)cr * 8) + up16((size_t)cc * 8) + 256;
  WDR_HIP(hipHostMalloc((void**)&h_, bytes_, hipHostMallocDefault));
  d_ = DevMem(bytes_);
  WDR_HIP(hipEventCreateWithFlags(&ev_, hipEventDisableTiming));
}

RowBatch::~RowBatch() {
  std::lock_guard<std::recursive_mutex> g(hip_alloc_mutex());
  if (pending_) (void)hipEventSynchronize(ev_);
  if (ev_) (void)hipEventDestroy(ev_);
  if (h_) (void)hipHostFree(h_);
}

void RowBatch::clear() {
  if (pending_) {
    WDR_HIP(hipEventSynchronize(ev_));
    pending_ = false;
  }
  R = n_logit = n_vgrp = vgrp_max = n_tiles = n_cap = 0;
  tok_.clear(); pos_.clear(); seq_.clear(); grp_.clear(); lend_.clear(); lead_.clear(); lrow_.clear();
  crow_.clear(); cstride_.clear(); tiles_.clear(); xkv_.clear(); cdst_.clear();
}

int RowBatch::add(const RowGroupDesc& g) {
  WDR_CHECK(g.n >= 1 && g.xkv && g.tok, "row batch: empty group");
  WDR_CHECK(R + g.n <= cap_rows, "row batch: rows over capacity");
  const int r0 = R;
  for (int i = 0; i < g.n; ++i) {
    tok_.push_back(g.tok[i]);
    pos_.push_back(g.pos ? g.pos[i] : g.pos0 + i);
    seq_.push_back(g.seq ? g.seq[i] : g.seq0);
    xkv_.push_back(g.xkv);
    grp_.push_back(0);
    lend_.push_back(kNoEnd);
  }
  R += g.n;
  if (g.n <= XATTN_GRP_MAX) {
    grp_[r0] = g.n;
    lend_[r0] = g.l_end;
    lead_.push_back(r0);
    n_vgrp++;
    vgrp_max = std::max(vgrp_max, g.n);
  } else {
    for (int t = 0; t < g.n; t += kTileRows) tiles_.push_back(make_int4(r0 + t, std::min(kTileRows, g.n - t), g.l_end, 0));
    n_tiles = (int)tiles_.size();
  }
  int first_logit = -1;
  if (g.logits) {
    first_logit = n_logit;
    for (int i = g.logits == 1 ? g.n - 1 : 0; i < g.n; ++i) lrow_.push_back(r0 + i);
    n_logit = (int)lrow_.size();
    WDR_CHECK(n_logit <= cap_logits, "row batch: logit rows over capacity");
  }
  if (g.cap) {
    for (int i = 0; i < g.n; ++i) {
      crow_.push_back(r0 + i);
      cdst_.push_back(g.cap + (size_t)i * XKV_T);
      cstride_.push_back(g.n * XKV_T);
    }
    n_cap = (int)crow_.size();
    WDR_CHECK(n_cap <= cap_caps, "row batch: capture rows over capacity");
  }
  return first_logit;
}

void RowBatch::upload(RowsIO& io, hipStream_t s, bool copy, bool track) {
  WDR_CHECK(R >= 1, "row batch: no rows");
  if (io.seq_stride > 0 && io.layer_stride > 0) {
    const long long nseq = io.layer_stride / io.seq_stride;
    for (int i = 0; i < R; ++i) WDR_CHECK(seq_[i] >= 0 && seq_[i] < nseq, "row batch: KV sequence outside the pool");
  }
  size_t off = 0;
  auto put = [&](const void* src, size_t n) -> const void* {
    const size_t o = off;
    if (n) memcpy(h_ + o, src, n);
    off = up16(off + n);
    WDR_CHECK(off <= bytes_, "row batch: tables over capacity");
    return (const void*)(d_.as<char>() + o);
  };
  io.tok = (const int*)put(tok_.data(), (size_t)R * 4);
  io.pos = (const int*)put(pos_.data(), (size_t)R * 4);
  io.seq = (const int*)put(seq_.data(), (size_t)R * 4);
  io.grp = (const int*)put(grp_.data(), (size_t)R * 4);
  io.lend = (const int*)put(lend_.data(), (size_t)R * 4);
  io.lead = (const int*)put(lead_.data(), lead_.size() * 4);
  io.lrow = (const int*)put(lrow_.data(), lrow_.size() * 4);
  io.crow = (const int*)put(crow_.data(), crow_.size() * 4);
  io.cstride = (const int*)put(cstride_.data(), cstride_.size() * 4);
  io.tiles = (const int4*)put(tiles_.data(), tiles_.size() * 16);
  io.xkv = (const f16* const*)put(xkv_.data(), (size_t)R * sizeof(void*));
  io.cdst = (float* const*)put(cdst_.data(), cdst_.size() * sizeof(void*));
  io.n_vgrp = n_vgrp;
  io.vgrp_max = std::max(1, vgrp_max);
  io.n_tiles = n_tiles;
  io.n_logit = n_logit;
  io.n_cap = n_cap;
  if (!copy) return;
  WDR_HIP(wdr_memcpy_async(d_.p, h_, off, hipMemcpyHostToDevice, s));
  if (track) {
    WDR_HIP(hipEventRecord(ev_, s));
    pending_ = true;
  }
}

void RowsBufs::alloc(int r, int lr, int d, int H, int V) {
  std::lock_guard<std::recursive_mutex> g(hip_alloc_mutex());
  rows = r;
  logit_rows = lr;
  xd = DevMem((size_t)r * d * 4);
  hd = DevMem((size_t)r * d * 2);
  qkvd = DevMem((size_t)r * 3 * d * 2);
  attd = DevMem((size_t)r * d * 2);
  qx = DevMem((size_t)r * d * 2);
  mlpd = DevMem((size_t)r * 4 * d * 2);
  part_o = DevMem((size_t)24 * r * H * 64 * 4);
  part_ml = DevMem((size_t)24 * r * H * sizeof(float2));
  ml = DevMem((size_t)r * H * sizeof(float2));
  logits = DevMem((size_t)std::max(1, lr) * V * 4);
}

RowsIO RowsBufs::io(const Context& ctx, int V) const {
  RowsIO o{};
  o.xd = xd.as<float>();
  o.hd = hd.as<f16>();
  o.qkvd = qkvd.as<f16>();
  o.attd = attd.as<f16>();
  o.qx = qx.as<f16>();
  o.mlpd = mlpd.as<f16>();
  o.part_o = part_o.as<float>();
  o.part_ml = part_ml.as<float2>();
  o.ml = ml.as<float2>();
  o.logits = logits.as<float>();
  o.ldlogits = V;
  o.kc = ctx.kv_k.as<f16>();
  o.vc = ctx.kv_v.as<f16>();
  o.layer_stride = ctx.kv_layer_stride;
  o.seq_stride = ctx.kv_seq_stride;
  return o;
}

void rows_forward(const Context& ctx, const RowsIO& io, int R, hipStream_t s, int l_stop) {
  const Model& md = ctx.model;
  const HParams& hp = md.hp;
  const int d = hp.n_text_state, L = hp.n_text_layer, H = hp.n_text_head;
  const float scale = 1.0f / 8.0f;
  WDR_CHECK(R >= 1 && io.tok && io.xkv, "rows forward: no rows / tables");
  static const int ln_env = getenv("WDR_ROWS_LN_FUSE") ? atoi(getenv("WDR_ROWS_LN_FUSE")) : -1;
  const int fuse_qkv = ln_env >= 0 ? ln_env : 48, fuse_xq = ln_env >= 0 ? ln_env : 64,
            fuse_fc1 = ln_env >= 0 ? ln_env : 24, fuse_logits = ln_env >= 0 ? ln_env : 0;
  auto P = [&](const f16* A, int lda, const f16* W, const float* b, void* out, int ldo, int N, int K, int epi,
               const float* lng = nullptr, const float* lnb = nullptr, int fuse_max = 0) {
    ProjArgs a{A, lda, W, K, b, out, ldo, nullptr, 0, R, N, K, epi};
    a.rows_mma = 1;
    if (lng) {
      if (R <= fuse_max) {
        a.ln_x = io.xd;
        a.ldln = d;
        a.ln_g = lng;
        a.ln_b = lnb;
      } else {
        launch_layernorm(io.xd, d, lng, lnb, io.hd, d, R, d, s);
        a.A = io.hd;
        a.lda = d;
      }
    }
    return a;
  };
  launch_embed(md.tok_emb, md.dec_pos, io.tok, io.pos, R, d, io.xd, s);
  const bool any_cap = io.n_cap > 0 && ctx.aheads_per_layer.size() == (size_t)L;
  int cap_slot0 = 0;
  for (int l = 0; l < L; ++l) {
    const DecLayer& e = md.dec[l];
    f16* kc = io.kc + (size_t)l * io.layer_stride;
    f16* vc = io.vc + (size_t)l * io.layer_stride;
    ProjArgs q = P(nullptr, d, e.w_qkv, e.b_qkv, io.qkvd, 3 * d, 3 * d, d, EPI_QKV_CACHE, e.ln1_g, e.ln1_b, fuse_qkv);
    q.kc = kc;
    q.vc = vc;
    q.seq_stride = io.seq_stride;
    q.row_seq = io.seq;
    q.row_pos = io.pos;
    q.d = d;
    launch_proj(q, s);
    DecSelfArgs sa{io.qkvd, 3 * d, kc, vc, io.seq_stride, d, io.seq, io.pos, io.attd, d, scale};
    launch_dec_self_attn(sa, R, H, s);
    launch_proj(P(io.attd, d, e.w_o, e.b_o, io.xd, d, d, d, EPI_F32_RESID), s);
    launch_proj(P(nullptr, d, e.w_xq, e.b_xq, io.qx, d, d, d, EPI_F16, e.ln2_g, e.ln2_b, fuse_xq), s);
    XAttnArgs xa{io.qx, d, nullptr, nullptr, 64, XKV_T, R, H, scale, io.part_o, io.part_ml, io.attd, d};
    xa.row_k = io.xkv;
    xa.layer_off = xkv_k_off(l, H);
    xa.v_off = xkv_v_off(l, H) - xkv_k_off(l, H);
    xa.hs = XKV_HS;
    xa.grp = io.grp;
    xa.lead = io.lead;
    xa.n_grp = io.n_vgrp;
    xa.n_vgrp = io.n_vgrp;
    xa.vgrp_max = io.vgrp_max;
    xa.lend = io.lend;
    xa.layer = l;
    xa.tiles = io.tiles;
    xa.n_tiles = io.n_tiles;
    const bool cap_layer = any_cap && !ctx.aheads_per_layer[l].empty();
    xa.ml_out = cap_layer ? io.ml : nullptr;
    launch_xattn_rows(xa, s);
    if (cap_layer) {
      CaptureRowsArgs ca{io.qx, d, io.xkv, xkv_k_off(l, H), XKV_HS, io.ml,
                         ctx.aheads_dev.as<int>() + ctx.aheads_dev_off[l], io.crow, io.cdst, io.cstride,
                         io.n_cap, cap_slot0, XKV_T, H, scale};
      launch_aheads_capture_rows(ca, (int)ctx.aheads_per_layer[l].size(), s);
    }
    if (ctx.aheads_per_layer.size() == (size_t)L) cap_slot0 += (int)ctx.aheads_per_layer[l].size();
    if (l + 1 >= l_stop) return;
    launch_proj(P(io.attd, d, e.w_xo, e.b_xo, io.xd, d, d, d, EPI_F32_RESID), s);
    launch_proj(P(nullptr, d, e.w_fc1, e.b_fc1, io.mlpd, 4 * d, 4 * d, d, EPI_F16_GELU, e.ln3_g, e.ln3_b, fuse_fc1), s);
    launch_proj(P(io.mlpd, 4 * d, e.w_fc2, e.b_fc2, io.xd, d, d, 4 * d, EPI_F32_RESID), s);
  }
  if (io.n_logit > 0) {
    ProjArgs a{nullptr, d, md.tok_emb, d, nullptr, io.logits, io.ldlogits, nullptr, 0, io.n_logit, hp.n_vocab, d, EPI_F32};
    a.rows_mma = 1;
    if (io.n_logit <= fuse_logits) {
      a.ln_x = io.xd;
      a.ldln = d;
      a.ln_g = md.ln_g;
      a.ln_b = md.ln_b;
      a.row_map = io.lrow;
    } else {
      launch_layernorm_rows(io.xd, d, md.ln_g, md.ln_b, io.hd, d, io.n_logit, d, io.lrow, s);
      a.A = io.hd;
    }
    launch_proj(a, s);
  }
}

void dtw_rows_forward(const Context& ctx, const RowsIO& io, int R, int l_end, hipStream_t s) {
  WDR_CHECK(io.n_cap == R && ctx.aheads_per_layer.size() == (size_t)ctx.model.hp.n_text_layer,
            "DTW rows forward: every row a capture row, alignment heads known");
  WDR_CHECK(l_end >= 1 && l_end <= ctx.model.hp.n_text_layer, "DTW rows forward: bad last layer");
  rows_forward(ctx, io, R, s, l_end);
}

}
```

whisper-diarize-rs_amd/csrc/whisper.h:

```cpp
#pragma once

#include <exception>
#include <atomic>
#include <memory>
#include <mutex>
#include <string>
#include <utility>
#include <vector>

#include "common.h"
#include "kernels/kernels.h"
#include "vocab.h"

namespace wdr {

uint64_t fnv1a64(const std::string& s);

struct HParams {
  int n_vocab = 51864, n_audio_ctx = 1500, n_audio_state = 512, n_audio_head = 8, n_audio_layer = 6;
  int n_text_ctx = 448, n_text_state = 512, n_text_head = 8, n_text_layer = 6, n_mels = 80;
};
bool hparams_for(const std::string& name, HParams* hp);

std::vector<std::pair<int, int>> alignment_heads_for(const std::string& model_name);

std::recursive_mutex& hip_alloc_mutex();
hipStream_t dedicated_stream(const char* knob, bool def, int prio);
void destroy_stream_pools();

struct DevMem {
  void* p = nullptr;
  size_t bytes = 0;
  DevMem() = default;
  explicit DevMem(size_t n);
  ~DevMem();
  DevMem(const DevMem&) = delete;
  DevMem& operator=(const DevMem&) = delete;
  DevMem(DevMem&& o) noexcept : p(o.p), bytes(o.bytes) { o.p = nullptr; o.bytes = 0; }
  DevMem& operator=(DevMem&& o) noexcept;
  template <typename T> T* as() const { return (T*)p; }
};

struct EncLayer {
  f16 *w_qkv, *w_o, *w_fc1, *w_fc2;
  float *b_qkv, *b_o, *b_fc1, *b_fc2, *ln1_g, *ln1_b, *ln2_g, *ln2_b;
};
struct DecLayer {
  f16 *w_qkv, *w_o, *w_xq, *w_xo, *w_fc1, *w_fc2;
  float *b_qkv, *b_o, *b_xq, *b_xo, *b_fc1, *b_fc2;
  float *ln1_g, *ln1_b, *ln2_g, *ln2_b, *ln3_g, *ln3_b;
};

struct Model {
  HParams hp;
  int kp1 = 0;
  f16 *conv1_w = nullptr, *conv2_w = nullptr;
  float *conv1_b = nullptr, *conv2_b = nullptr, *enc_pos = nullptr, *ln_post_g = nullptr, *ln_post_b = nullptr;
  std::vector<EncLayer> enc;
  std::vector<DecLayer> dec;
  f16* w_xkv = nullptr;
  float* b_xkv = nullptr;
  f16* tok_emb = nullptr;
  float *dec_pos = nullptr, *ln_g = nullptr, *ln_b = nullptr;
  float *mel_filters = nullptr, *hann = nullptr, *cos_tab = nullptr, *sin_tab = nullptr;
  DevMem storage;
  size_t weight_bytes = 0;
};

std::vector<uint8_t> fp8_plan_for(int n_layer);

struct ContextParams {
  bool use_gpu = true;
  int gpu_device = 0;
  bool dtw = true;
  bool flash_attn = false;
  double weight_std = 0.02;
  double emb_std = 0.02;
};

class Context {
 public:
  Context(const std::string& model_name, const HParams& hp, const ContextParams& cp,
          const class GgmlFile* gf = nullptr);
  ~Context();
  std::string name;
  ContextParams cp;
  Model model;
  Vocab vocab;
  std::vector<std::pair<int, int>> aheads;
  std::vector<std::vector<int>> aheads_per_layer;
  DevMem aheads_dev;
  std::vector<int> aheads_dev_off;
  hipStream_t stream = nullptr;
  hipStream_t low_prime = nullptr;
  std::vector<hipStream_t> prime_streams;
  int max_chains = 1;
  DevMem kv_k, kv_v;
  long long kv_seq_stride = 0, kv_layer_stride = 0;
  std::vector<std::unique_ptr<class StepBatcher>> batchers;
  int n_batchers = 1;
  StepBatcher& step_batcher(int chain = 0);
  std::unique_ptr<class StepBatcher> prefill_b;
  bool prefill_split = false;
  StepBatcher& prefill_batcher();
  std::unique_ptr<class DtwQueue> dtwq;
  class DtwQueue& dtw_queue();
  struct BatchStats {
    long long launches = 0, rows = 0, prefill_rows = 0, dtw_rows = 0, prefills = 0, dtws = 0, mixed = 0;
    long long vgroups = 0, tiles = 0;
    double step_s = 0;
    long long dq_passes = 0, dq_rows = 0, dq_jobs = 0;
  };
  BatchStats batcher_stats();
  std::atomic<bool> fp8_encoder{false};
  std::vector<uint8_t> fp8_plan;
  enum { F8_QKV = 1, F8_O = 2, F8_FC1 = 4, F8_FC2 = 8 };
  struct Fp8W {
    DevMem w, s;
  };
  struct Fp8Layer {
    Fp8W qkv, o, fc1, fc2;
  };
  const std::vector<Fp8Layer>& fp8_layers();

 private:
  std::mutex fp8_mu_;
  std::vector<Fp8Layer> fp8_layers_;
  void fp8_build();
};

struct FullParams {
  bool greedy = false;
  int best_of = 5, beam_size = 5;
  std::string language = "auto";
  bool translate = false;
  int n_max_text_ctx = 16384;
  std::string initial_prompt;
  bool has_initial_prompt = false;
  float temperature = 0.f, temperature_inc = 0.2f;
  float entropy_thold = 2.4f, logprob_thold = -1.f, no_speech_thold = 0.6f;
  float thold_pt = 0.01f, thold_ptsum = 0.01f, max_initial_ts = 1.f, length_penalty = -1.f;
  bool suppress_blank = true, single_segment = true, token_timestamps = true;
  int max_tokens = 0;
  float force_len_rate = 0.f;
};

struct TokenData {
  int id = 0, tid = 0;
  float p = 0, plog = 0, pt = 0, ptsum = 0;
  long long t0 = -1, t1 = -1, t_dtw = -1;
  float vlen = 0;
};

struct ResultSeg {
  long long t0, t1;
  std::string text;
  std::vector<TokenData> tokens;
};

struct StageTimes {
  double mel = 0, encode = 0, decode = 0, dtw = 0, glue = 0;
  long long windows = 0, decode_steps = 0, prefills = 0;
  double lang = 0, prompt_gpu = 0;
  long long lang_passes = 0, lang_rows = 0;
};

class StepBatcher {
 public:
  explicit StepBatcher(Context& ctx);
  ~StepBatcher();
  static constexpr int kRows = 8;
  struct Req {
    int n = 1;
    int tok[kRows], seq[kRows], pos[kRows];
    LogitsCtl ctl[kRows];
    const f16* xkv = nullptr;
    VocabIds vids{};
    int K = 0;
    TokenData out[kRows];
    BeamCand cand[kRows * BEAM_KMAX];
    int pn = 0;
    const int* ptok = nullptr;
    int pseq = 0;
    const f16* pxkv = nullptr;
    LogitsCtl pctl{};
    TokenData pout;
    float pnosp = 0.f;
    BeamCand pcand[BEAM_KMAX];
    int dn = 0;
    const int* dtok = nullptr;
    int dseq = 0;
    const f16* dxkv = nullptr;
    float* dcap = nullptr;
    int dl_end = 1 << 30;
    int ln = 0;
    int lseq = 0;
    const f16* lxkv = nullptr;
    float lout[100];
    bool done = false;
    std::exception_ptr err;
  };
  void enter();
  void leave();
  void step(Req& r);
  void run(std::vector<Req*>& batch) { launch(batch); }
  long long launches = 0, rows = 0, prefill_rows = 0, dtw_rows = 0, prefills = 0, dtws = 0, mixed = 0;
  long long vgroups = 0, tiles = 0;
  double step_s = 0;
  struct Impl;

 private:
  Context& ctx_;
  std::unique_ptr<Impl> m_;
  void launch(std::vector<Req*>& batch);
};
// ... 121 lines not shown
```

whisper-diarize-rs_amd/csrc/whisper_ctx.cpp:

```cpp
#include "whisper.h"
#include "rows.h"
#include "ggml_file.h"
#include "prof.h"

#include <algorithm>
#include <functional>
#include <chrono>
#include <cmath>
#include <cstring>
#include <cstdlib>
#include <map>
#include <random>
#include <exception>
#include <condition_variable>
#include <deque>
#include <set>
#include <pthread.h>
#include <thread>
#include <mutex>
#include <sstream>

namespace wdr {

static double now_s() {
// ... 362 lines not shown
  m.weight_bytes = A.off;
  m.storage = DevMem(A.off);
  char* base = m.storage.as<char>();
  auto h16 = [&](size_t o) { return (f16*)(base + o); };
  auto f32 = [&](size_t o) { return (float*)(base + o); };
  m.conv1_w = h16(o_c1w); m.conv1_b = f32(o_c1b); m.conv2_w = h16(o_c2w); m.conv2_b = f32(o_c2b);
  m.enc_pos = f32(o_epos); m.ln_post_g = f32(o_lnpg); m.ln_post_b = f32(o_lnpb);
  for (auto& e : eo)
    m.enc.push_back({h16(e.qkv), h16(e.o), h16(e.f1), h16(e.f2), f32(e.bqkv), f32(e.bo), f32(e.bf1), f32(e.bf2),
                     f32(e.l1g), f32(e.l1b), f32(e.l2g), f32(e.l2b)});
  for (auto& e : dd)
    m.dec.push_back({h16(e.qkv), h16(e.o), h16(e.xq), h16(e.xo), h16(e.f1), h16(e.f2), f32(e.bqkv), f32(e.bo),
                     f32(e.bxq), f32(e.bxo), f32(e.bf1), f32(e.bf2), f32(e.l1g), f32(e.l1b), f32(e.l2g), f32(e.l2b),
                     f32(e.l3g), f32(e.l3b)});
  m.w_xkv = h16(o_xkv); m.b_xkv = f32(o_bxkv); m.tok_emb = h16(o_tok); m.dec_pos = f32(o_dpos);
  m.ln_g = f32(o_lng); m.ln_b = f32(o_lnb);
  m.mel_filters = f32(o_filt); m.hann = f32(o_hann); m.cos_tab = f32(o_cos); m.sin_tab = f32(o_sin);

  hipStream_t s = stream;
  const double sq3 = std::sqrt(3.0);
  DevMem qstage;
  if (gf) {
    size_t mx = 0;
    for (const auto& kv : gf->tensors)
      if (kv.second.quantized()) mx = std::max(mx, kv.second.n_bytes());
    if (mx) qstage = DevMem((mx + 3) & ~size_t(3));
  }
  auto fill = [&](void* dst, const std::string& nm, long long rows, int src_cols, int dst_cols, bool is16, double sd) {
    if (!gf) {
      launch_synth_fill(dst, rows, src_cols, dst_cols, fnv1a64(nm), (float)(sd * sq3), is16, 0, 0.f, s);
      return;
    }
    const int64_t n = rows * (int64_t)src_cols;
    if (is16 && gf->get(nm).quantized()) {
      const GgmlTensor& t = gf->get(nm);
      WDR_CHECK(t.n_elem() == n, "failed to open model: tensor '" + nm + "' has " + std::to_string(t.n_elem()) +
                                     " elements, expected " + std::to_string(n));
      WDR_CHECK(dst_cols == src_cols, "ggml load: padded quantized tensor '" + nm + "'");
      WDR_CHECK(t.n_bytes() <= qstage.bytes, "ggml load: quantized staging buffer too small");
      WDR_HIP(hipMemcpy(qstage.p, t.data, t.n_bytes(), hipMemcpyHostToDevice));
      launch_dequant(t.type, qstage.p, n / 32, (f16*)dst, s);
      WDR_HIP(hipStreamSynchronize(s));
      return;
    }
    if (is16) {
      std::vector<uint16_t> v = gf->as_f16(nm, n), padded;
      if (dst_cols != src_cols) {
        padded.assign((size_t)rows * dst_cols, 0);
        for (long long r = 0; r < rows; ++r) memcpy(&padded[r * dst_cols], &v[r * src_cols], (size_t)src_cols * 2);
        v.swap(padded);
      }
      WDR_HIP(hipMemcpy(dst, v.data(), v.size() * 2, hipMemcpyHostToDevice));
    } else {
      WDR_CHECK(dst_cols == src_cols, "ggml load: padded f32 tensor");
      const std::vector<float> v = gf->as_f32(nm, n);
      WDR_HIP(hipMemcpy(dst, v.data(), v.size() * 4, hipMemcpyHostToDevice));
    }
  };
  auto cfill = [&](float* dst, long long n, float v) { launch_synth_fill(dst, 1, (int)n, (int)n, 0, 0.f, false, 1, v, s); };
  auto lnfill = [&](float* dst, const std::string& nm, long long n, float v) {
    if (gf) fill(dst, nm, 1, (int)n, (int)n, false, 0.0);
    else cfill(dst, n, v);
  };
  const double sd = cp.weight_std;
  fill(m.conv1_w, "encoder.conv1.weight", d, hp.n_mels * 3, m.kp1, true, sd);
  fill(m.conv1_b, "encoder.conv1.bias", 1, d, d, false, sd);
  fill(m.conv2_w, "encoder.conv2.weight", d, 3 * d, 3 * d, true, sd);
  fill(m.conv2_b, "encoder.conv2.bias", 1, d, d, false, sd);
  fill(m.enc_pos, "encoder.positional_embedding", hp.n_audio_ctx, d, d, false, sd);
  for (int i = 0; i < hp.n_audio_layer; ++i) {
    const std::string p = "encoder.blocks." + std::to_string(i) + ".";
    const EncLayer& e = m.enc[i];
    fill(e.w_qkv, p + "attn.query.weight", d, d, d, true, sd);
    fill(e.w_qkv + (size_t)d * d, p + "attn.key.weight", d, d, d, true, sd);
    fill(e.w_qkv + (size_t)2 * d * d, p + "attn.value.weight", d, d, d, true, sd);
    fill(e.b_qkv, p + "attn.query.bias", 1, d, d, false, sd);
    cfill(e.b_qkv + d, d, 0.f);
    fill(e.b_qkv + 2 * d, p + "attn.value.bias", 1, d, d, false, sd);
    fill(e.w_o, p + "attn.out.weight", d, d, d, true, sd);
    fill(e.b_o, p + "attn.out.bias", 1, d, d, false, sd);
    fill(e.w_fc1, p + "mlp.0.weight", 4 * d, d, d, true, sd);
    fill(e.b_fc1, p + "mlp.0.bias", 1, 4 * d, 4 * d, false, sd);
    fill(e.w_fc2, p + "mlp.2.weight", d, 4 * d, 4 * d, true, sd);
    fill(e.b_fc2, p + "mlp.2.bias", 1, d, d, false, sd);
    lnfill(e.ln1_g, p + "attn_ln.weight", d, 1.f); lnfill(e.ln1_b, p + "attn_ln.bias", d, 0.f);
    lnfill(e.ln2_g, p + "mlp_ln.weight", d, 1.f); lnfill(e.ln2_b, p + "mlp_ln.bias", d, 0.f);
  }
  lnfill(m.ln_post_g, "encoder.ln_post.weight", d, 1.f);
  lnfill(m.ln_post_b, "encoder.ln_post.bias", d, 0.f);
  fill(m.tok_emb, "decoder.token_embedding.weight", hp.n_vocab, dt, dt, true, cp.emb_std);
  fill(m.dec_pos, "decoder.positional_embedding", hp.n_text_ctx, dt, dt, false, sd);
  for (int i = 0; i < L; ++i) {
    const std::string p = "decoder.blocks." + std::to_string(i) + ".";
    const DecLayer& e = m.dec[i];
    fill(e.w_qkv, p + "attn.query.weight", dt, dt, dt, true, sd);
    fill(e.w_qkv + (size_t)dt * dt, p + "attn.key.weight", dt, dt, dt, true, sd);
    fill(e.w_qkv + (size_t)2 * dt * dt, p + "attn.value.weight", dt, dt, dt, true, sd);
    fill(e.b_qkv, p + "attn.query.bias", 1, dt, dt, false, sd);
    cfill(e.b_qkv + dt, dt, 0.f);
    fill(e.b_qkv + 2 * dt, p + "attn.value.bias", 1, dt, dt, false, sd);
    fill(e.w_o, p + "attn.out.weight", dt, dt, dt, true, sd);
    fill(e.b_o, p + "attn.out.bias", 1, dt, dt, false, sd);
    fill(e.w_xq, p + "cross_attn.query.weight", dt, dt, dt, true, sd);
    fill(e.b_xq, p + "cross_attn.query.bias", 1, dt, dt, false, sd);
    fill(m.w_xkv + (size_t)i * 2 * dt * d, p + "cross_attn.key.weight", dt, d, d, true, sd);
    fill(m.w_xkv + (size_t)(i * 2 + 1) * dt * d, p + "cross_attn.value.weight", dt, d, d, true, sd);
    cfill(m.b_xkv + (size_t)i * 2 * dt, dt, 0.f);
    fill(m.b_xkv + (size_t)(i * 2 + 1) * dt, p + "cross_attn.value.bias", 1, dt, dt, false, sd);
    fill(e.w_xo, p + "cross_attn.out.weight", dt, dt, dt, true, sd);
    fill(e.b_xo, p + "cross_attn.out.bias", 1, dt, dt, false, sd);
    fill(e.w_fc1, p + "mlp.0.weight", 4 * dt, dt, dt, true, sd);
    fill(e.b_fc1, p + "mlp.0.bias", 1, 4 * dt, 4 * dt, false, sd);
    fill(e.w_fc2, p + "mlp.2.weight", dt, 4 * dt, 4 * dt, true, sd);
    fill(e.b_fc2, p + "mlp.2.bias", 1, dt, dt, false, sd);
    lnfill(e.ln1_g, p + "attn_ln.weight", dt, 1.f); lnfill(e.ln1_b, p + "attn_ln.bias", dt, 0.f);
    lnfill(e.ln2_g, p + "cross_attn_ln.weight", dt, 1.f); lnfill(e.ln2_b, p + "cross_attn_ln.bias", dt, 0.f);
    lnfill(e.ln3_g, p + "mlp_ln.weight", dt, 1.f); lnfill(e.ln3_b, p + "mlp_ln.bias", dt, 0.f);
  }
  lnfill(m.ln_g, "decoder.ln.weight", dt, 1.f);
  lnfill(m.ln_b, "decoder.ln.bias", dt, 0.f);
  std::vector<float> filt = mel_filters_host(hp.n_mels), hann(400), cs(400), sn(400);
  if (gf) {
    WDR_CHECK(gf->n_mel == hp.n_mels && gf->n_fft == 201, "ggml load: mel filter bank shape");
    filt = gf->filters;
    for (size_t i = 0; i < gf->vocab.size() && (int)i < vocab.n_vocab; ++i) vocab.id_to_token[i] = gf->vocab[i];
    vocab.token_to_id.clear();
    for (int i = 0; i < vocab.n_vocab; ++i) vocab.token_to_id[vocab.id_to_token[i]] = i;
  }
  for (int i = 0; i < 400; ++i) {
    hann[i] = (float)(0.5 * (1.0 - std::cos(2.0 * M_PI * i / 400.0)));
    cs[i] = (float)std::cos(2.0 * M_PI * i / 400.0);
    sn[i] = (float)(-std::sin(2.0 * M_PI * i / 400.0));
  }
  WDR_HIP(wdr_memcpy_async(m.mel_filters, filt.data(), filt.size() * 4, hipMemcpyHostToDevice, s));
  WDR_HIP(wdr_memcpy_async(m.hann, hann.data(), 1600, hipMemcpyHostToDevice, s));
  WDR_HIP(wdr_memcpy_async(m.cos_tab, cs.data(), 1600, hipMemcpyHostToDevice, s));
  WDR_HIP(wdr_memcpy_async(m.sin_tab, sn.data(), 1600, hipMemcpyHostToDevice, s));

  if (cp.dtw) {
    aheads = alignment_heads_for(name);
    aheads_per_layer.assign(L, {});
    for (auto& a : aheads) {
      WDR_CHECK(a.first < L && a.second < hp.n_text_head, "alignment head out of range for this model");
      aheads_per_layer[a.first].push_back(a.second);
    }
    std::vector<int> flat;
    for (int l = 0; l < L; ++l) {
      aheads_dev_off.push_back((int)flat.size());
      for (int h : aheads_per_layer[l]) flat.push_back(h);
    }
    aheads_dev = DevMem(std::max<size_t>(4, flat.size() * 4));
    if (!flat.empty()) WDR_HIP(wdr_memcpy_async(aheads_dev.p, flat.data(), flat.size() * 4, hipMemcpyHostToDevice, s));
  }
  WDR_HIP(hipStreamSynchronize(s));
  qstage = DevMem();
  {
    const char* e = getenv("WDR_DECODE_CHAINS");
    max_chains = std::max(1, std::min(64, e ? atoi(e) : 40));
    const char* nb = getenv("WDR_BATCHERS");
    n_batchers = std::max(1, std::min(8, nb ? atoi(nb) : 1));
    prefill_split = getenv("WDR_PREFILL_SPLIT") && atoi(getenv("WDR_PREFILL_SPLIT")) != 0;
    fp8_encoder = getenv("WDR_FP8_ENCODER") && atoi(getenv("WDR_FP8_ENCODER")) != 0;
    fp8_plan = fp8_plan_for(hp.n_audio_layer);
    const size_t per = (size_t)hp.n_text_layer * 21 * hp.n_text_ctx * hp.n_text_state;
    kv_k = DevMem(per * max_chains * 2);
    kv_v = DevMem(per * max_chains * 2);
    kv_seq_stride = (long long)hp.n_text_ctx * hp.n_text_state;
    kv_layer_stride = (long long)max_chains * 21 * kv_seq_stride;
  }
  if (getenv("WDR_DTWQ_EARLY") && atoi(getenv("WDR_DTWQ_EARLY")) != 0 && !aheads.empty()) {
    DtwQueue& q = dtw_queue();
    (void)q;
  }
}

Context::~Context() {
  dtwq.reset();
  batchers.clear();
  prefill_b.reset();
  if (stream) (void)hipStreamDestroy(stream);
  if (low_prime) (void)hipStreamDestroy(low_prime);
  for (hipStream_t ps : prime_streams) (void)hipStreamDestroy(ps);
}

static constexpr int RMAX = 448;
static constexpr int NSEQ = 8;
static constexpr int NSLOT = 21;
static constexpr int DTW_SEQ = 16;
static constexpr int LANG_SEQ = 17;


struct State::Impl {
  int d, L, H, V, n_mels, kp1;
  struct EncBufs {
    int nb = 0;
    DevMem im2col, c1, ex, eh, eqkv, eatt, emlp;
    DevMem q8a, qsa, q8m, qsm;
  };
  EncBufs eb, e1;
  struct Slot {
    DevMem x, mel, gmax, pcm;
    int16_t* h_pcm = nullptr;
    DevMem energy_d;
    float* h_energy = nullptr;
    int energy_cap = 0, energy_n = -1;
    int pcm_cap = 0, x_cap = 0, mel_cap = 0, n_fft_frames = 0, n_samples = 0;
    hipEvent_t ready = nullptr, freed = nullptr;
    std::shared_ptr<DtwQJob> dtw;
  };
  std::vector<Slot> slots;
  int S = 0;
  DevMem xkv_ring;
  size_t xkv_slot_elems = 0;
  int cur = 0;
  bool own_shared = false;
  bool es_shared = false;
  hipStream_t es = nullptr;
  struct Plan {
    std::vector<const int16_t*> pcm;
    std::vector<int> n;
    size_t next_enq = 0;
    bool detect_lang = false;
  } plan;
  RowsBufs lb;
  std::unique_ptr<RowBatch> tlb;
  struct EncGraph {
    hipGraphExec_t exec = nullptr;
    std::unique_ptr<RowBatch> tl;
  };
  std::map<int, EncGraph> enc_graphs;
  hipStream_t es_cap = nullptr;
  std::atomic<long long> t_fence{0}, t_enc_launch{0};
  std::thread enc_th;
  std::mutex enc_mu;
  std::condition_variable enc_cv;
  int enc_target = -1;
  bool enc_stop = false, enc_busy = false;
  std::exception_ptr enc_err;
  std::atomic<long long> enc_windows{0};
  std::atomic<long long> lang_passes{0}, lang_rows{0};
  float* h_lang = nullptr;
  std::vector<int> lang_src;
  std::function<bool(StepBatcher::Req&)> lang_ride;
  std::function<void(const StepBatcher::Req&)> lang_after;
  DevMem energy_d; int energy_cap = 0;
  const f16* xkv() const { return xkv_ring.as<f16>() + (size_t)(xsel >= 0 ? S + 1 : cur) * xkv_slot_elems; }
  int xsel = -1;
  std::shared_ptr<DtwQJob> alt_dtw;
  RowsBufs mb, db;
  std::unique_ptr<RowBatch> tb, tdb;
  DevMem work, tokout, ctl, cap;
  DevMem beamc, kvpairs;
  BeamCand* h_beam = nullptr;
  DevMem sprobs, slogp;
  std::vector<float> hp_probs, hp_logp;
  std::mt19937 rng[NSEQ];
  int* h_pairs = nullptr;
  f16* kc = nullptr;
  f16* vc = nullptr;
  int nslot_tot = 0;
  long long seq_stride = 0;
  hipStream_t own = nullptr;
  hipStream_t eo = nullptr;
  bool eo_shared = false;
  DevMem nrm, xdtw, times;
  struct DtwSet {
    DevMem cap, nrm, xdtw, times;
  } dset;
  hipStream_t sd = nullptr;
  hipEvent_t ev_sync = nullptr;
  hipEvent_t ev_dtw = nullptr;
  hipEvent_t ev_p0 = nullptr, ev_p1 = nullptr;
  struct DtwJob {
    int i0 = 0, n = 0;
    int* blk = nullptr;
    hipEvent_t done = nullptr;
    std::shared_ptr<DtwQJob> q;
  };
  std::vector<std::shared_ptr<DtwQJob>> qlive;
  std::vector<DtwJob> jobs;
  struct PendingDtw {
    bool on = false;
    std::vector<int> toks;
    const f16* xkv = nullptr;
    int slot = -1;
    int sot_len = 0, seek = 0, n_audio = 0;
    int* blk = nullptr;
    hipEvent_t done = nullptr;
  } pend;
  std::vector<int*> blk_pool;
  std::vector<hipEvent_t> ev_pool;
  TokOut* h_tok = nullptr;
  LogitsCtl* h_ctl = nullptr;
  int* h_times = nullptr;
  VocabIds vids;
  struct StepGraph {
    hipGraphExec_t exec = nullptr;
    VocabIds vids{};
  };
  std::map<int, StepGraph> graphs;
};

std::vector<uint8_t> fp8_plan_for(int n_layer) {
  std::vector<uint8_t> plan(n_layer, 0xf);
  if (const char* e = getenv("WDR_FP8_PLAN"); e && *e) {
    uint8_t last = 0xf;
    for (int l = 0; l < n_layer; ++l) {
      if (e[l] && isxdigit((unsigned char)e[l])) {
// ... 2699 lines not shown
```

whisper-diarize-rs_amd/wdr/__init__.py:

```python
from __future__ import annotations

import ctypes as C
import dataclasses
import enum
from typing import Callable, List, Optional

import numpy as np

from . import _lib as L

__all__ = ["Engine", "EngineConfig", "TranscribeOptions", "AdvancedTranscribe", "DiarizeOptions", "Segment",
           "WordTimestamp",
           "ProgressType", "Callbacks", "Synthetic", "WhisperContext", "SpeechSegment", "read_wav", "vad_merge",
           "WdrError"]

WdrError = L.WdrError


class ProgressType(enum.IntEnum):
    Download = 0
    Transcribe = 1
    Translate = 2


# ... 490 lines not shown
        return (cls, lp.reshape(nw, 589, 7)) if logprobs else cls

    def get_segments(self, samples: np.ndarray, materialize: bool = True):
        smp = np.ascontiguousarray(samples, np.int16)
        sp, ns = C.POINTER(L.SpeechSegment)(), C.c_size_t()
        L.check(self._lib.wdr_diarize_get_segments(self.h, smp.ctypes.data_as(C.POINTER(C.c_int16)), smp.size,
                                                   C.byref(sp), C.byref(ns)))
        try:
            if not materialize:
                return [(sp[i].start, sp[i].end) for i in range(ns.value)]
            return [SpeechSegment(sp[i].start, sp[i].end, np.ctypeslib.as_array(sp[i].samples, (sp[i].n_samples,)).copy()
                                  if sp[i].n_samples else np.zeros(0, np.int16)) for i in range(ns.value)]
        finally:
            self._lib.wdr_free(C.cast(sp, C.c_void_p))

    @staticmethod
    def segments_from_classes(cls: np.ndarray, samples: np.ndarray):
        smp = np.ascontiguousarray(samples, np.int16)
        c = np.ascontiguousarray(cls, np.int32)
        sp, ns = C.POINTER(L.SpeechSegment)(), C.c_size_t()
        lib = L.load()
        L.check(lib.wdr_diarize_segments_from_classes(c.ctypes.data_as(C.POINTER(C.c_int32)), c.shape[0],
                                                      smp.ctypes.data_as(C.POINTER(C.c_int16)), smp.size,
                                                      C.byref(sp), C.byref(ns)))
        try:
            return [SpeechSegment(sp[i].start, sp[i].end, np.ctypeslib.as_array(sp[i].samples, (sp[i].n_samples,)).copy()
                                  if sp[i].n_samples else np.zeros(0, np.int16)) for i in range(ns.value)]
        finally:
            lib.wdr_free(C.cast(sp, C.c_void_p))

    def fbank(self, samples: np.ndarray) -> np.ndarray:
        smp = np.ascontiguousarray(samples, np.int16)
        out = np.zeros((smp.size // 160 + 1, 80), np.float32)
        nf = C.c_size_t()
        L.check(self._lib.wdr_diarize_fbank(self.h, smp.ctypes.data_as(C.POINTER(C.c_int16)), smp.size,
                                            out.ctypes.data_as(C.POINTER(C.c_float)), C.byref(nf)))
        return out[:nf.value]

    def embedding(self, samples: np.ndarray):
        smp = np.ascontiguousarray(samples, np.int16)
        out = np.zeros(512, np.float32)
        ok = C.c_int8()
        L.check(self._lib.wdr_diarize_embedding(self.h, smp.ctypes.data_as(C.POINTER(C.c_int16)), smp.size,
                                                out.ctypes.data_as(C.POINTER(C.c_float)), C.byref(ok)))
        return out if ok.value else None

    def embedding_batch(self, segments):
        smp = [np.ascontiguousarray(x, np.int16) for x in segments]
        B = len(smp)
        ptrs = (C.POINTER(C.c_int16) * max(B, 1))(*[x.ctypes.data_as(C.POINTER(C.c_int16)) for x in smp])
        ns = (C.c_size_t * max(B, 1))(*[x.size for x in smp])
        out = np.zeros((max(B, 1), 512), np.float32)
        ok = (C.c_int8 * max(B, 1))()
        L.check(self._lib.wdr_diarize_embedding_batch(self.h, ptrs, ns, B, out.ctypes.data_as(C.POINTER(C.c_float)), ok))
        return [out[b].copy() if ok[b] else None for b in range(B)]

    def stats(self):
        a, b = C.c_double(), C.c_double()
        L.check(self._lib.wdr_diarize_stats(self.h, C.byref(a), C.byref(b)))
        return a.value, b.value

    def __del__(self):
        try:
            self._lib.wdr_diarizer_free(self.h)
        except Exception:
            pass


def model_file_tensors(kind: str, path: str) -> dict:
    lib = L.load()
    k = {"silero": 0, "segmentation": 1, "campplus": 2}[kind]
    names, data, n = C.c_void_p(), C.POINTER(C.c_float)(), C.c_size_t()
    L.check(lib.wdr_dbg_model_file(k, path.encode(), C.byref(names), C.byref(data), C.byref(n)))
    try:
        txt = C.cast(names, C.c_char_p).value.decode()
        flat = np.ctypeslib.as_array(data, (max(1, n.value),))[:n.value].copy()
    finally:
        lib.wdr_free(names)
        lib.wdr_free(C.cast(data, C.c_void_p))
    out, o = {}, 0
    for line in txt.splitlines():
        name, cnt = line.rsplit(":", 1)
        out[name] = flat[o:o + int(cnt)]
        o += int(cnt)
    return out


def ggml_info(path: str) -> dict:
    lib = L.load()
    hp = (C.c_int32 * 11)()
    nt, nv = C.c_int64(), C.c_int64()
    L.check(lib.wdr_ggml_info(path.encode(), hp, C.byref(nt), C.byref(nv)))
    keys = ["n_vocab", "n_audio_ctx", "n_audio_state", "n_audio_head", "n_audio_layer", "n_text_ctx",
            "n_text_state", "n_text_head", "n_text_layer", "n_mels", "ftype"]
    counts = (C.c_int64 * 16)()
    L.check(lib.wdr_ggml_tensor_types(path.encode(), counts))
    ftype = hp[10]
    return {**dict(zip(keys, list(hp))), "n_tensors": nt.value, "n_vocab_tokens": nv.value,
            "ftype_base": ftype % 1000, "qnt_version": ftype // 1000,
            "tensor_types": {i: int(c) for i, c in enumerate(counts) if c}}


GGML_QUANT_TYPES = {"q4_0": 2, "q4_1": 3, "q5_0": 6, "q5_1": 7, "q8_0": 8}
GGML_BLOCK_BYTES = {2: 18, 3: 20, 6: 22, 7: 24, 8: 34}


def ggml_tensor_f16(path: str, name: str) -> np.ndarray:
    lib = L.load()
    out, n = C.POINTER(C.c_uint16)(), C.c_size_t()
    L.check(lib.wdr_ggml_tensor_f16(path.encode(), name.encode(), C.byref(out), C.byref(n)))
    try:
        return np.ctypeslib.as_array(out, (max(1, n.value),))[:n.value].copy().view(np.float16)
    finally:
        lib.wdr_free(C.cast(out, C.c_void_p))


def dbg_dequant(fmt, blocks, timing: bool = False):
    lib = L.load()
    t = GGML_QUANT_TYPES.get(fmt, fmt)
    raw = np.ascontiguousarray(np.frombuffer(bytes(blocks), np.uint8) if not isinstance(blocks, np.ndarray)
                               else blocks.astype(np.uint8, copy=False).ravel())
    bs = GGML_BLOCK_BYTES[t]
    if raw.size % bs:
        raise ValueError("%d bytes are not whole %d-byte blocks" % (raw.size, bs))
    nb = raw.size // bs
    out = np.empty(nb * 32, np.uint16)
    ms = C.c_double()
    L.check(lib.wdr_dbg_dequant(t, raw.ctypes.data_as(C.POINTER(C.c_uint8)), nb,
                                out.ctypes.data_as(C.POINTER(C.c_uint16)), C.byref(ms) if timing else None))
    return (out.view(np.float16), ms.value) if timing else out.view(np.float16)


_U16P, _I32P, _F32P = C.POINTER(C.c_uint16), C.POINTER(C.c_int32), C.POINTER(C.c_float)


def _h16(a):
    return np.ascontiguousarray(np.asarray(a).astype(np.float16)).view(np.uint16)


def dbg_self_attn(q, kc, vc, row_seq, row_pos, n_head: int) -> np.ndarray:
    qb, kb, vb = _h16(q), _h16(kc), _h16(vc)
    rs, rp = np.ascontiguousarray(row_seq, np.int32), np.ascontiguousarray(row_pos, np.int32)
    R, d = qb.shape
    n_seq, T, dk = kb.shape
    if d != 64 * n_head or dk != d or vb.shape != kb.shape or rs.shape != (R,) or rp.shape != (R,):
        raise ValueError("dbg_self_attn: q [R][64 H], kc / vc [n_seq][T][64 H], row_seq / row_pos [R]")
    out = np.zeros((R, d), np.float32)
    L.check(L.load().wdr_dbg_self_attn(qb.ctypes.data_as(_U16P), kb.ctypes.data_as(_U16P), vb.ctypes.data_as(_U16P),
                                       n_seq, T, rs.ctypes.data_as(_I32P), rp.ctypes.data_as(_I32P), R, n_head,
                                       out.ctypes.data_as(_F32P)))
    return out


def dbg_proj_qkv(a, w, bias, row_seq, row_pos, kc, vc):
    ab, wb = _h16(a), _h16(w)
    M, K = ab.shape
    d = wb.shape[0] // 3
    kb, vb = _h16(kc).copy(), _h16(vc).copy()
    n_seq, T, dk = kb.shape
    rs, rp = np.ascontiguousarray(row_seq, np.int32), np.ascontiguousarray(row_pos, np.int32)
    if wb.shape != (3 * d, K) or dk != d or vb.shape != kb.shape or rs.shape != (M,) or rp.shape != (M,):
        raise ValueError("dbg_proj_qkv: a [M][K], w [3 d][K], kc / vc [n_seq][T][d], row_seq / row_pos [M]")
    b = None if bias is None else np.ascontiguousarray(bias, np.float32)
    q = np.zeros((M, d), np.float32)
    L.check(L.load().wdr_dbg_proj_qkv(ab.ctypes.data_as(_U16P), wb.ctypes.data_as(_U16P),
                                      None if b is None else b.ctypes.data_as(_F32P), M, d, K,
                                      rs.ctypes.data_as(_I32P), rp.ctypes.data_as(_I32P), n_seq, T,
                                      kb.ctypes.data_as(_U16P), vb.ctypes.data_as(_U16P), q.ctypes.data_as(_F32P)))
    return q, kb.view(np.float16), vb.view(np.float16)


class WhisperContext:

    def __init__(self, model_name: str, model_path: Optional[str] = None, gpu_device: Optional[int] = None,
                 use_gpu: Optional[bool] = None, enable_dtw: Optional[bool] = True,
                 enable_flash_attn: Optional[bool] = None, num_samples: Optional[int] = None,
                 synthetic: Optional[Synthetic] = None):
        lib = L.load()
        self._lib = lib
        h = C.c_void_p()
        syn = _syn(synthetic)
        L.check(lib.wdr_context_create(_s(model_path), model_name.encode(), 0 if gpu_device is None else 1,
                                       gpu_device or 0, _ob(use_gpu), _ob(enable_dtw), _ob(enable_flash_attn),
                                       0 if num_samples is None else 1, num_samples or 0,
                                       C.byref(syn) if syn else None, C.byref(h)))
        self.h = h
        self.synthetic = synthetic
        hp = (C.c_int32 * 10)()
        L.check(lib.wdr_context_hparams(h, hp))
        keys = ["n_vocab", "n_audio_ctx", "n_audio_state", "n_audio_head", "n_audio_layer", "n_text_ctx",
                "n_text_state", "n_text_head", "n_text_layer", "n_mels"]
        self.hparams = dict(zip(keys, list(hp)))

    def close(self):
        if self.h:
            self._lib.wdr_context_free(self.h)
            self.h = None

    def __del__(self):
        try:
            self.close()
        except Exception:
            pass

    def run_pipeline(self, speech_segments, options: TranscribeOptions, callbacks: Optional[Callbacks] = None,
                     synthetic: Optional[Synthetic] = None, with_index: bool = False,
                     diarize_options: Optional[DiarizeOptions] = None):
        keep = _Keep()
        arr = (L.SpeechSegment * max(1, len(speech_segments)))()
        for i, s in enumerate(speech_segments):
            smp = keep(np.ascontiguousarray(s.samples, np.int16))
            arr[i] = L.SpeechSegment(s.start, s.end, smp.ctypes.data_as(C.POINTER(C.c_int16)), smp.size)
        out = C.POINTER(L.SegmentList)()
        syn = _syn(synthetic or self.synthetic)
        d = _dopts(diarize_options, keep)
        L.check(self._lib.wdr_run_pipeline(self.h, arr, len(speech_segments), _opts(options, keep),
                                           C.byref(d) if d is not None else None,
                                           C.byref(syn) if syn else None, _callbacks(callbacks, keep),
                                           C.byref(out)))
        return _segments(out, with_index)

    def run_pipeline_raw(self, speech_segments, options: TranscribeOptions, synthetic: Optional[Synthetic] = None):
        keep = _Keep()
        arr = (L.SpeechSegment * max(1, len(speech_segments)))()
        for i, s in enumerate(speech_segments):
            smp = keep(np.ascontiguousarray(s.samples, np.int16))
            arr[i] = L.SpeechSegment(s.start, s.end, smp.ctypes.data_as(C.POINTER(C.c_int16)), smp.size)
        out = C.POINTER(L.SegmentList)()
        syn = _syn(synthetic or self.synthetic)
        L.check(self._lib.wdr_run_pipeline_raw(self.h, arr, len(speech_segments), _opts(options, keep),
                                               C.byref(syn) if syn else None, C.byref(out)))
        segs, lang, index = _segments(out, True)
        return segs, lang, index or []

    def run_pipeline_block(self, speech_segments, options: TranscribeOptions, rng_in: Optional[str] = None,
                           synthetic: Optional[Synthetic] = None):
        keep = _Keep()
        arr = (L.SpeechSegment * max(1, len(speech_segments)))()
        for i, s in enumerate(speech_segments):
            smp = keep(np.ascontiguousarray(s.samples, np.int16))
            arr[i] = L.SpeechSegment(s.start, s.end, smp.ctypes.data_as(C.POINTER(C.c_int16)), smp.size)
        out = C.POINTER(L.SegmentList)()
        syn = _syn(synthetic or self.synthetic)
        sampled = (C.c_int8 * max(1, len(speech_segments)))()
        rng = C.c_void_p()
        L.check(self._lib.wdr_run_pipeline_block(self.h, arr, len(speech_segments), _opts(options, keep),
                                                 C.byref(syn) if syn else None, _s(rng_in), sampled, C.byref(rng),
                                                 C.byref(out)))
        rng_out = C.cast(rng, C.c_char_p).value.decode()
        self._lib.wdr_free(rng)
        segs, lang, index = _segments(out, True)
        return segs, lang, index or [], [bool(sampled[i]) for i in range(len(speech_segments))], rng_out

    @property
    def devices(self) -> List[int]:
        n = C.c_int32()
        ids = (C.c_int32 * 8)()
        L.check(self._lib.wdr_context_devices(self.h, C.byref(n), ids, 8))
        return [ids[i] for i in range(min(n.value, 8))]

    def set_encoder_fp8(self, on: bool):
        L.check(self._lib.wdr_context_set_encoder_fp8(self.h, 1 if on else 0))

    def set_chains(self, n: int):
        L.check(self._lib.wdr_context_set_chains(self.h, int(n)))

    def set_early_fixup(self, mode: int):
        L.check(self._lib.wdr_dbg_set_early_fixup(self.h, int(mode)))

    def stage_times(self) -> dict:
        t = L.StageTimes()
        L.check(self._lib.wdr_context_stage_times(self.h, C.byref(t)))
        return {f: getattr(t, f) for f, _ in L.StageTimes._fields_}

    def state_full(self, samples_f32: np.ndarray, options: TranscribeOptions, initial_prompt: Optional[str] = None,
                   synthetic: Optional[Synthetic] = None):
        keep = _Keep()
        x = np.ascontiguousarray(samples_f32, np.float32)
        segs = C.POINTER(L.ResultSeg)()
        n = C.c_size_t()
        lang = C.c_int32()
        syn = _syn(synthetic or self.synthetic)
        L.check(self._lib.wdr_state_full(self.h, x.ctypes.data_as(C.POINTER(C.c_float)), x.size, _opts(options, keep),
                                         C.byref(syn) if syn else None, _s(initial_prompt), C.byref(segs), C.byref(n),
                                         C.byref(lang)))
        out = []
        for i in range(n.value):
            s = segs[i]
            toks = [dict(id=t.id, tid=t.tid, p=t.p, plog=t.plog, pt=t.pt, ptsum=t.ptsum, t0=t.t0, t1=t.t1,
                         t_dtw=t.t_dtw) for t in (s.tokens[k] for k in range(s.n_tokens))]
            out.append(dict(t0=s.t0, t1=s.t1, text=s.text.decode(), tokens=toks))
        self._lib.wdr_result_free(segs, n.value)
        return out, lang.value

    def log_mel_window(self, x: np.ndarray, seek: int = 0) -> np.ndarray:
        x = np.ascontiguousarray(x, np.float32)
        out = np.zeros((self.hparams["n_mels"], 3000), np.float32)
        L.check(self._lib.wdr_dbg_log_mel(self.h, x.ctypes.data_as(C.POINTER(C.c_float)), x.size, seek,
                                          out.ctypes.data_as(C.POINTER(C.c_float))))
        return out

    def encode(self, mel_window: np.ndarray) -> np.ndarray:
        m = np.ascontiguousarray(mel_window, np.float32)
        out = np.zeros((1500, self.hparams["n_audio_state"]), np.float32)
        L.check(self._lib.wdr_dbg_encode(self.h, m.ctypes.data_as(C.POINTER(C.c_float)),
                                         out.ctypes.data_as(C.POINTER(C.c_float))))
        return out

    def cross_kv(self) -> np.ndarray:
        h = self.hparams
        out = np.zeros((1500, h["n_text_layer"], 2, h["n_text_state"]), np.float32)
        L.check(self._lib.wdr_dbg_cross_kv(self.h, out.ctypes.data_as(C.POINTER(C.c_float))))
        return out

    def decode(self, tokens) -> np.ndarray:
        t = np.ascontiguousarray(tokens, np.int32)
        out = np.zeros(self.hparams["n_vocab"], np.float32)
        L.check(self._lib.wdr_dbg_decode(self.h, t.ctypes.data_as(C.POINTER(C.c_int32)), t.size,
                                         out.ctypes.data_as(C.POINTER(C.c_float))))
        return out

# ... 142 lines not shown
```

whisper-diarize-rs_amd/wdr/_lib.py:

```python
from __future__ import annotations

import atexit
import ctypes as C
import os
import re

PKG_DIR = os.path.dirname(os.path.dirname(os.path.abspath(__file__)))
LIB_PATH = os.environ.get("WDR_AB_LIB") or os.path.join(PKG_DIR, "libwdr.so")
HEADER = os.path.join(os.path.dirname(PKG_DIR), "include", "wdr.h")

i8, i32, i64, u64 = C.c_int8, C.c_int32, C.c_int64, C.c_uint64
f32, f64, cstr, vp, sz = C.c_float, C.c_double, C.c_char_p, C.c_void_p, C.c_size_t


class EngineConfig(C.Structure):
    _fields_ = [("cache_dir", cstr), ("enable_dtw", i8), ("enable_flash_attn", i8), ("use_gpu", i8),
                ("has_gpu_device", i8), ("gpu_device", i32), ("vad_model_path", cstr),
                ("diarize_segment_model_path", cstr), ("diarize_embedding_model_path", cstr)]


class Advanced(C.Structure):
    _fields_ = [("sampling_strategy", cstr), ("has_best_of_or_beam_size", i8), ("best_of_or_beam_size", i32),
                ("has_n_threads", i8), ("n_threads", i32), ("has_temperature", i8), ("temperature", f32),
                ("has_max_text_ctx", i8), ("max_text_ctx", i32), ("init_prompt", cstr),
# ... 17 lines not shown

class FormattingOverrides(C.Structure):
    _fields_ = [("has_max_chars_per_line", i8), ("max_chars_per_line", u64), ("has_max_lines", i8),
                ("max_lines", u64), ("has_cps_cap", i8), ("cps_cap", f64), ("has_split_gap_sec", i8),
                ("split_gap_sec", f64), ("has_comma_min_chars_before_allow", i8),
                ("comma_min_chars_before_allow", u64), ("has_min_word_dur", i8), ("min_word_dur", f64),
                ("has_min_sub_dur", i8), ("min_sub_dur", f64), ("has_max_sub_dur", i8), ("max_sub_dur", f64),
                ("has_soft_max_words_per_line", i8), ("soft_max_words_per_line", u64),
                ("insert_interword_space", i8), ("use_grapheme_len", i8), ("enforce_kinsoku", i8),
                ("allow_comma_split", i8)]


class Word(C.Structure):
    _fields_ = [("text", cstr), ("start", f64), ("end", f64), ("has_probability", i8), ("probability", f32)]


class Segment(C.Structure):
    _fields_ = [("start", f64), ("end", f64), ("text", cstr), ("words", C.POINTER(Word)), ("n_words", sz),
                ("speaker_id", cstr)]


class SegmentList(C.Structure):
    _fields_ = [("segments", C.POINTER(Segment)), ("n_segments", sz), ("detected_lang", cstr),
                ("speech_index", C.POINTER(C.c_int64))]


class SpeechSegment(C.Structure):
    _fields_ = [("start", f64), ("end", f64), ("samples", C.POINTER(C.c_int16)), ("n_samples", sz)]


PROGRESS_FN = C.CFUNCTYPE(None, vp, i32, i32, cstr)
SEGMENT_FN = C.CFUNCTYPE(None, vp, C.POINTER(Segment))
CANCEL_FN = C.CFUNCTYPE(C.c_int, vp)


class Callbacks(C.Structure):
    _fields_ = [("user", vp), ("progress", PROGRESS_FN), ("new_segment", SEGMENT_FN), ("is_cancelled", CANCEL_FN)]


class StageTimes(C.Structure):
    _fields_ = [("mel", f64), ("encode", f64), ("decode", f64), ("dtw", f64), ("vad", f64), ("total", f64),
                ("windows", i64), ("decode_steps", i64), ("prefills", i64), ("lang", f64), ("prompt_gpu", f64),
                ("embed", f64), ("chains", i64), ("batch_launches", i64), ("batch_rows", i64),
                ("fixup_segments", i64), ("replay_segments", i64), ("spec_s", f64), ("fixup_s", f64),
                ("batch_step_s", f64), ("early_fixup_segments", i64), ("batch_prefill_rows", i64),
                ("batch_dtw_rows", i64), ("batch_prefills", i64), ("batch_dtws", i64), ("batch_mixed", i64),
                ("batch_xattn_groups", i64), ("batch_xattn_tiles", i64), ("dtwq_passes", i64), ("dtwq_rows", i64),
                ("dtwq_jobs", i64), ("lang_passes", i64), ("lang_rows", i64)]


class Token(C.Structure):
    _fields_ = [("id", i32), ("tid", i32), ("p", f32), ("plog", f32), ("pt", f32), ("ptsum", f32),
                ("t0", i64), ("t1", i64), ("t_dtw", i64)]


class ResultSeg(C.Structure):
    _fields_ = [("t0", i64), ("t1", i64), ("text", cstr), ("tokens", C.POINTER(Token)), ("n_tokens", sz)]


P = C.POINTER
_SIGS = {
    "wdr_last_error": (cstr, []),
    "wdr_abi_version": (C.c_int, []),
    "wdr_device_count": (C.c_int, []),
    "wdr_shutdown": (None, []),
    "wdr_engine_new": (C.c_int, [P(EngineConfig), P(vp)]),
    "wdr_engine_free": (None, [vp]),
    "wdr_engine_set_synthetic": (C.c_int, [vp, P(Synthetic)]),
    "wdr_transcribe_audio": (C.c_int, [vp, cstr, P(TranscribeOptions), P(FormattingOverrides), P(Callbacks),
                                       P(P(SegmentList))]),
    "wdr_read_wav": (C.c_int, [cstr, P(P(C.c_int16)), P(sz)]),
    "wdr_audio_info": (C.c_int, [cstr, P(i32), P(u64)]),
    "wdr_read_audio": (C.c_int, [cstr, i8, i32, P(P(C.c_int16)), P(sz)]),
    "wdr_engine_set_audio_convert": (C.c_int, [vp, i8]),
    "wdr_dbg_audio_convert": (C.c_int, [P(C.c_uint8), u64, i32, i32, i32, u64, i32, P(P(C.c_int16)), P(sz), P(f64)]),
    "wdr_read_audio_channels": (C.c_int, [cstr, i8, i32, P(P(C.c_int16)), P(sz), P(i32)]),
    "wdr_dbg_audio_split": (C.c_int, [P(C.c_uint8), u64, i32, i32, i32, u64, i32, P(P(C.c_int16)), P(sz), P(f64)]),
    "wdr_engine_set_channel_split": (C.c_int, [vp, i8]),
    "wdr_dbg_resample_table": (C.c_int, [i32, P(i32), P(i32), P(i32), P(P(f32))]),
    "wdr_dbg_model_file": (C.c_int, [i32, cstr, P(C.c_void_p), P(P(f32)), P(sz)]),
    "wdr_process_segments": (C.c_int, [P(Segment), sz, cstr, P(FormattingOverrides), i8, P(f64), sz,
                                       P(P(SegmentList))]),
    "wdr_free": (None, [vp]),
    "wdr_vad_merge": (C.c_int, [P(f64), P(f64), sz, P(C.c_int16), sz, P(f64), P(sz), P(f64), P(i64), P(sz)]),
    "wdr_vad_create": (C.c_int, [cstr, i8, i32, P(vp)]),
    "wdr_vad_free": (None, [vp]),
    "wdr_vad_probs": (C.c_int, [vp, P(C.c_int16), sz, P(f32), P(f64)]),
    "wdr_vad_stats": (C.c_int, [vp, P(f64)]),
    "wdr_vad_segments_from_probs": (C.c_int, [P(f32), sz, P(f32), P(sz)]),
    "wdr_vad_get_segments": (C.c_int, [vp, P(C.c_int16), sz, P(P(f64)), P(sz), P(P(SpeechSegment)), P(sz)]),
    "wdr_diarizer_create": (C.c_int, [cstr, cstr, i8, i32, P(vp)]),
    "wdr_diarizer_free": (None, [vp]),
    "wdr_diarize_frame_classes": (C.c_int, [vp, P(C.c_int16), sz, P(i32), P(f32)]),
    "wdr_diarize_get_segments": (C.c_int, [vp, P(C.c_int16), sz, P(P(SpeechSegment)), P(sz)]),
    "wdr_diarize_segments_from_classes": (C.c_int, [P(i32), sz, P(C.c_int16), sz, P(P(SpeechSegment)), P(sz)]),
    "wdr_diarize_fbank": (C.c_int, [vp, P(C.c_int16), sz, P(f32), P(sz)]),
    "wdr_diarize_embedding": (C.c_int, [vp, P(C.c_int16), sz, P(f32), P(i8)]),
    "wdr_diarize_embedding_batch": (C.c_int, [vp, P(P(C.c_int16)), P(sz), i32, P(f32), P(i8)]),
    "wdr_diarize_stats": (C.c_int, [vp, P(f64), P(f64)]),
    "wdr_speakers_new": (C.c_int, [i8, u64, P(vp)]),
    "wdr_speakers_free": (None, [vp]),
    "wdr_speakers_assign": (C.c_int, [vp, P(f32), i32, f32, C.c_char_p, sz]),
    "wdr_context_create": (C.c_int, [cstr, cstr, i8, i32, i8, i8, i8, i8, u64, P(Synthetic), P(vp)]),
    "wdr_context_free": (None, [vp]),
    "wdr_run_pipeline_raw": (C.c_int, [vp, P(SpeechSegment), sz, P(TranscribeOptions), P(Synthetic),
                                       P(P(SegmentList))]),
    "wdr_run_pipeline": (C.c_int, [vp, P(SpeechSegment), sz, P(TranscribeOptions), P(DiarizeOptions), P(Synthetic),
                                   P(Callbacks), P(P(SegmentList))]),
    "wdr_run_pipeline_block": (C.c_int, [vp, P(SpeechSegment), sz, P(TranscribeOptions), P(Synthetic), cstr, P(i8),
                                         P(C.c_void_p), P(P(SegmentList))]),
    "wdr_segment_list_free": (None, [P(SegmentList)]),
    "wdr_context_set_chains": (C.c_int, [vp, i32]),
    "wdr_context_devices": (C.c_int, [vp, P(i32), P(i32), i32]),
    "wdr_context_set_encoder_fp8": (C.c_int, [vp, C.c_int8]),
    "wdr_dbg_set_early_fixup": (C.c_int, [vp, i32]),
    "wdr_dbg_set_gemm32": (C.c_int, [i32]),
    "wdr_ggml_info": (C.c_int, [cstr, P(i32), P(i64), P(i64)]),
    "wdr_ggml_tensor_types": (C.c_int, [cstr, P(i64)]),
    "wdr_ggml_tensor_f16": (C.c_int, [cstr, cstr, P(P(C.c_uint16)), P(sz)]),
    "wdr_dbg_dequant": (C.c_int, [i32, P(C.c_uint8), sz, P(C.c_uint16), P(f64)]),
    "wdr_dbg_batch_step": (C.c_int, [vp, P(i32), sz, i32, i32, P(f64)]),
    "wdr_context_stage_times": (C.c_int, [vp, P(StageTimes)]),
    "wdr_context_hparams": (C.c_int, [vp, P(i32)]),
    "wdr_prof_set": (C.c_int, [i32]),
    "wdr_prof_read": (C.c_int, [P(f64), P(i64), P(f64), P(f64)]),
    "wdr_prof_set_mask": (C.c_int, [i32]),
    "wdr_prof_read_class": (C.c_int, [i32, P(f64), P(i64), P(f64), P(f64)]),
    "wdr_prof_read_clock": (C.c_int, [i32, P(f64), P(i64), P(f64), P(f64)]),
    "wdr_state_full": (C.c_int, [vp, P(f32), sz, P(TranscribeOptions), P(Synthetic), cstr, P(P(ResultSeg)), P(sz),
                                 P(i32)]),
    "wdr_result_free": (None, [P(ResultSeg), sz]),
    "wdr_dbg_log_mel": (C.c_int, [vp, P(f32), sz, i32, P(f32)]),
    "wdr_dbg_energy": (C.c_int, [P(f32), sz, P(f32)]),
    "wdr_dbg_mfma_scale": (C.c_int, [P(C.c_uint8), P(C.c_uint8), P(i32), P(i32), P(f32)]),
    "wdr_dbg_encode": (C.c_int, [vp, P(f32), P(f32)]),
    "wdr_dbg_decode": (C.c_int, [vp, P(i32), sz, P(f32)]),
    "wdr_dbg_cross_kv": (C.c_int, [vp, P(f32)]),
    "wdr_dbg_step": (C.c_int, [vp, P(i32), sz, P(f32)]),
    "wdr_dbg_logits": (C.c_int, [vp, P(f32), i32, P(i32), P(f32), f32, i32, P(i32), P(f32)]),
    "wdr_dbg_capture": (C.c_int, [vp, P(i32), sz, P(f32)]),
    "wdr_dbg_dtw": (C.c_int, [P(f32), i32, i32, i32, i32, i32, P(f32), P(i32), P(i32)]),
    "wdr_dbg_discrete": (C.c_int, [P(f32), sz, C.c_uint32, i32, P(i32)]),
    "wdr_dbg_dtw_dp": (C.c_int, [P(f32), i32, i32, i32, P(i32), P(i32)]),
    "wdr_dbg_proj": (C.c_int, [P(C.c_uint16), P(C.c_uint16), P(f32), i32, i32, i32, i32, P(f32)]),
    "wdr_dbg_proj_ln": (C.c_int, [P(f32), P(f32), P(f32), P(C.c_uint16), P(f32), i32, i32, i32, i32, i32, P(f32)]),
    "wdr_dbg_proj_fp8": (C.c_int, [P(C.c_uint16), P(C.c_uint16), P(f32), i32, i32, i32, i32, P(f32), P(C.c_uint8),
                                   P(C.c_uint8), P(C.c_uint8), P(C.c_uint8)]),
    "wdr_dbg_attn": (C.c_int, [P(C.c_uint16), P(C.c_uint16), P(C.c_uint16), i32, i32, i32, i32, P(f32)]),
    "wdr_dbg_xattn": (C.c_int, [P(C.c_uint16), P(C.c_uint16), P(i32), P(i32), i32, i32, i32, i32, P(f32)]),
    "wdr_dbg_self_attn": (C.c_int, [P(C.c_uint16), P(C.c_uint16), P(C.c_uint16), i32, i32, P(i32), P(i32), i32, i32,
                                    P(f32)]),
    "wdr_dbg_proj_qkv": (C.c_int, [P(C.c_uint16), P(C.c_uint16), P(f32), i32, i32, i32, P(i32), P(i32), i32, i32,
                                   P(C.c_uint16), P(C.c_uint16), P(f32)]),
    "wdr_dbg_logits_topk": (C.c_int, [vp, P(f32), i32, P(i32), P(f32), f32, i32, i32, P(i32), P(f32)]),
    "wdr_dbg_logits_probs": (C.c_int, [vp, P(f32), i32, P(i32), P(f32), f32, i32, P(f32), P(f32)]),
    "wdr_dbg_kv_rows": (C.c_int, [vp, i32, i32, i32, P(C.c_uint16), P(C.c_uint16)]),
    "wdr_dbg_kv_reorder": (C.c_int, [vp, P(i32), P(i32), i32, i32]),
}

_lib = None


class WdrError(RuntimeError):
    pass


def header_symbols():
    txt = open(HEADER).read()
    return sorted(set(re.findall(r"\b(wdr_[a-z0-9_]+)\s*\(", txt)))


def load():
    global _lib
    if _lib is not None:
        return _lib
    if not os.path.exists(LIB_PATH):
        raise WdrError("libwdr.so not built at %s (run __graft_entry__.build())" % LIB_PATH)
    lib = C.CDLL(LIB_PATH)
    for name, (res, args) in _SIGS.items():
        fn = getattr(lib, name)
        fn.restype = res
        fn.argtypes = args
    _lib = lib
    atexit.register(lib.wdr_shutdown)
    return lib


def check(rc: int):
    if rc != 0:
        raise WdrError(load().wdr_last_error().decode("utf-8", "replace"))
```

Measured before the change: 873.1.

## Pack decoder row-projection weights in MFMA fragment order at load time

```diff
diff --git a/include/wdr.h b/include/wdr.h
--- a/include/wdr.h
+++ b/include/wdr.h
@@ -250,6 +250,8 @@
                  int32_t epi, float* out );
 #define WDR_DBG_PROJ_ROWS 0x200
 #define WDR_DBG_PROJ_GEMM1 0x800
+#define WDR_DBG_PROJ_PACKED 0x1000
+int wdr_dbg_pack_rows(const uint16_t* w_f16, int32_t N, int32_t K, uint16_t* out);
 int wdr_dbg_proj_ln(const float* x, const float* gamma, const float* beta, const uint16_t* w_f16, const float* bias,
                     int32_t M, int32_t N, int32_t K, int32_t epi, int32_t fused, float* out);
 int wdr_dbg_attn(const uint16_t* q, const uint16_t* k, const uint16_t* v, int32_t Tq, int32_t Tk, int32_t n_head,
@@ -262,6 +264,9 @@
 int wdr_dbg_proj_qkv(const uint16_t* a_f16, const uint16_t* w_f16, const float* bias, int32_t M, int32_t d, int32_t K,
                      const int32_t* row_seq, const int32_t* row_pos, int32_t n_seq, int32_t T, uint16_t* kc_io,
                      uint16_t* vc_io, float* q_out);
+int wdr_dbg_proj_qkv_packed(const uint16_t* a_f16, const uint16_t* w_f16, const float* bias, int32_t M, int32_t d,
+                            int32_t K, const int32_t* row_seq, const int32_t* row_pos, int32_t n_seq, int32_t T,
+                            uint16_t* kc_io, uint16_t* vc_io, float* q_out);
 int wdr_dbg_logits_topk(wdr_context* c, const float* logits, int32_t R, const int32_t* ctl, const float* temperature,
                         float max_initial_ts, int32_t suppress_blank, int32_t K, int32_t* ids_out, float* f_out);
 int wdr_dbg_logits_probs(wdr_context* c, const float* logits, int32_t R, const int32_t* ctl, const float* temperature,
diff --git a/whisper-diarize-rs_amd/csrc/common.h b/whisper-diarize-rs_amd/csrc/common.h
--- a/whisper-diarize-rs_amd/csrc/common.h
+++ b/whisper-diarize-rs_amd/csrc/common.h
@@ -93,6 +93,7 @@
   int tile_gm = 0;
   int gemm_ref = 0;
   int rows_mma = 0;
+  int b_packed = 0;
   const int* row_map = nullptr;
 };
 
@@ -114,6 +115,8 @@
 inline unsigned long long* prof_attach(A&) { return nullptr; }
 inline unsigned long long* prof_attach(ProjArgs& a) { return a.ts = prof_slot(); }
 void launch_proj(const ProjArgs& a, hipStream_t s);
+size_t packed_rows_elems(int N, int K);
+void launch_pack_rows(const f16* w, f16* out, int N, int K, hipStream_t s);
 void gemm_knobs_reload();
 void launch_proj_fp8(const ProjArgs& a, hipStream_t s);
 void launch_quant_f8(const f16* x, int ldx, int rows, int K, uint8_t* y, int ldy, uint32_t* sc, int ld_sc,
diff --git a/whisper-diarize-rs_amd/csrc/engine.cpp b/whisper-diarize-rs_amd/csrc/engine.cpp
--- a/whisper-diarize-rs_amd/csrc/engine.cpp
+++ b/whisper-diarize-rs_amd/csrc/engine.cpp
@@ -2409,6 +2409,27 @@
   })
 }
 
+static void dbg_pack(ProjArgs& a, bool packed, DevMem& pk) {
+  if (!packed) return;
+  WDR_CHECK(a.K >= 32 && a.K % 32 == 0, "dbg projection, packed weights: K % 32");
+  pk = DevMem(packed_rows_elems(a.N, a.K) * 2);
+  launch_pack_rows(a.B, pk.as<f16>(), a.N, a.K, nullptr);
+  a.B = pk.as<f16>();
+  a.b_packed = 1;
+}
+
+int wdr_dbg_pack_rows(const uint16_t* w16, int32_t N, int32_t K, uint16_t* out) {
+  WDR_GUARD({
+    WDR_CHECK(w16 && out && N >= 1 && N <= (1 << 20) && K >= 32 && K <= 8192 && K % 32 == 0, "dbg_pack_rows: bad shape (K % 32)");
+    DevMem dw((size_t)N * K * 2), dp(packed_rows_elems(N, K) * 2);
+    WDR_HIP(hipMemcpy(dw.p, w16, dw.bytes, hipMemcpyHostToDevice));
+    launch_pack_rows(dw.as<f16>(), dp.as<f16>(), N, K, nullptr);
+    WDR_HIP(hipDeviceSynchronize());
+    WDR_HIP(hipMemcpy(out, dp.p, dp.bytes, hipMemcpyDeviceToHost));
+    return 0;
+  })
+}
+
 int wdr_dbg_proj(const uint16_t* a16, const uint16_t* w16, const float* bias, int32_t M, int32_t N, int32_t K,
                  int32_t epi, float* out) {
   WDR_GUARD({
@@ -2420,13 +2441,16 @@
     const bool rows = (epi & 0x200) != 0;
     if (epi & 0x400) return fail("WDR_DBG_PROJ_SPLIT: the split-K residual projections were removed (k_skinny runs them whole)");
     const bool gemm_ref = (epi & 0x800) != 0;
+    const bool packed = (epi & 0x1000) != 0;
     epi &= 0xff;
     const bool f16out = epi == EPI_F16 || epi == EPI_F16_GELU;
     std::vector<f16> h16;
     if (!f16out) WDR_HIP(hipMemcpy(dout.p, out, dout.bytes, hipMemcpyHostToDevice));
     ProjArgs a{da.as<f16>(), K, dw.as<f16>(), K, bias ? db.as<float>() : nullptr, dout.p, N, nullptr, 0, M, N, K, epi};
-    a.rows_mma = rows ? 1 : 0;
+    a.rows_mma = rows || packed ? 1 : 0;
     a.gemm_ref = gemm_ref ? 1 : 0;
+    DevMem dpk;
+    dbg_pack(a, packed, dpk);
     launch_proj(a, nullptr);
     WDR_HIP(hipDeviceSynchronize());
     if (f16out) {
@@ -2454,6 +2478,16 @@
     if (bias) WDR_HIP(hipMemcpy(db.p, bias, db.bytes, hipMemcpyHostToDevice));
     ProjArgs a{nullptr, K, dw.as<f16>(), K, bias ? db.as<float>() : nullptr, dout.p, N, nullptr, 0, M, N, K, epi};
     a.rows_mma = 1;
+    DevMem dpk, dmap;
+    dbg_pack(a, (fused & 2) != 0, dpk);
+    if (fused & 4) {
+      std::vector<int> rm(M);
+      for (int m = 0; m < M; ++m) rm[m] = M - 1 - m;
+      dmap = DevMem((size_t)M * 4);
+      WDR_HIP(hipMemcpy(dmap.p, rm.data(), dmap.bytes, hipMemcpyHostToDevice));
+      a.row_map = dmap.as<int>();
+    }
+    fused &= 1;
     if (fused) {
       a.ln_x = dx.as<float>();
       a.ldln = K;
@@ -2614,9 +2648,9 @@
   })
 }
 
-int wdr_dbg_proj_qkv(const uint16_t* a16, const uint16_t* w16, const float* bias, int32_t M, int32_t d, int32_t K,
-                     const int32_t* row_seq, const int32_t* row_pos, int32_t n_seq, int32_t T, uint16_t* kc_io,
-                     uint16_t* vc_io, float* q_out) {
+static int dbg_proj_qkv(const uint16_t* a16, const uint16_t* w16, const float* bias, int32_t M, int32_t d, int32_t K,
+                        const int32_t* row_seq, const int32_t* row_pos, int32_t n_seq, int32_t T, uint16_t* kc_io,
+                        uint16_t* vc_io, float* q_out, bool packed) {
   WDR_GUARD({
     WDR_CHECK(a16 && w16 && row_seq && row_pos && kc_io && vc_io && q_out, "dbg qkv projection: null argument");
     WDR_CHECK(M >= 1 && M <= 4096 && d >= 64 && d <= 2048 && d % 64 == 0 && d % 8 == 0 && K >= 32 && K <= 8192 &&
@@ -2646,6 +2680,8 @@
     a.row_seq = ds.as<int>();
     a.row_pos = dp.as<int>();
     a.d = d;
+    DevMem dpk;
+    dbg_pack(a, packed, dpk);
     launch_proj(a, nullptr);
     WDR_HIP(hipDeviceSynchronize());
     std::vector<f16> h((size_t)M * d);
@@ -2655,6 +2691,16 @@
     WDR_HIP(hipMemcpy(vc_io, dv.p, cache, hipMemcpyDeviceToHost));
     return 0;
   })
+}
+int wdr_dbg_proj_qkv(const uint16_t* a16, const uint16_t* w16, const float* bias, int32_t M, int32_t d, int32_t K,
+                     const int32_t* row_seq, const int32_t* row_pos, int32_t n_seq, int32_t T, uint16_t* kc_io,
+                     uint16_t* vc_io, float* q_out) {
+  return dbg_proj_qkv(a16, w16, bias, M, d, K, row_seq, row_pos, n_seq, T, kc_io, vc_io, q_out, false);
+}
+int wdr_dbg_proj_qkv_packed(const uint16_t* a16, const uint16_t* w16, const float* bias, int32_t M, int32_t d,
+                            int32_t K, const int32_t* row_seq, const int32_t* row_pos, int32_t n_seq, int32_t T,
+                            uint16_t* kc_io, uint16_t* vc_io, float* q_out) {
+  return dbg_proj_qkv(a16, w16, bias, M, d, K, row_seq, row_pos, n_seq, T, kc_io, vc_io, q_out, true);
 }
 
 static void dbg_ctls(const int32_t* ctl, const float* temperature, int R, std::vector<LogitsCtl>& lc) {
diff --git a/whisper-diarize-rs_amd/csrc/kernels/gemm.hip b/whisper-diarize-rs_amd/csrc/kernels/gemm.hip
--- a/whisper-diarize-rs_amd/csrc/kernels/gemm.hip
+++ b/whisper-diarize-rs_amd/csrc/kernels/gemm.hip
@@ -1287,7 +1287,7 @@
   return std::max((uint32_t)16 * MT * K * 2, skinny_red_bytes<EPI, MT, NT, W>());
 }
 
-template <int EPI, int MT, int NT, int W = 4, bool LN = false, int UU = 0>
+template <int EPI, int MT, int NT, int W = 4, bool LN = false, int UU = 0, bool PK = false>
 __global__ __launch_bounds__(W * 64) void k_skinny(ProjArgs a) {
   ProfClock prof_clock_(a.ts);
   __shared__ float red_s[LN ? 1 : W * MT * NT * 4 * 64];
@@ -1360,9 +1360,14 @@
   const f16* brow[NT];
 #pragma unroll
   for (int j = 0; j < NT; ++j) {
-    int n = n0 + j * 16 + fr;
-    n = n < a.N ? n : a.N - 1;
-    brow[j] = a.B + (size_t)n * a.ldb + fk;
+    if constexpr (PK) {
+      const int strip = min((int)blockIdx.x * NT + j, cdiv(a.N, 16) - 1);
+      brow[j] = a.B + (size_t)strip * a.K * 16 + lane * 8;
+    } else {
+      int n = n0 + j * 16 + fr;
+      n = n < a.N ? n : a.N - 1;
+      brow[j] = a.B + (size_t)n * a.ldb + fk;
+    }
   }
   constexpr int U = UU > 0 ? UU : (MT + NT) <= 3 ? 8 : 4;
   for (int k0 = wid * 32; k0 < a.K; k0 += 32 * W * U) {
@@ -1374,7 +1379,7 @@
       const int kk = ok ? k : 0;
 #pragma unroll
       for (int j = 0; j < NT; ++j) {
-        const f16x8 t = *(const f16x8*)(brow[j] + kk);
+        const f16x8 t = *(const f16x8*)(brow[j] + (PK ? kk * 16 : kk));
         bf[u][j] = ok ? t : (f16x8){};
       }
 #pragma unroll
@@ -1507,48 +1512,78 @@
   const bool ln = a.ln_x != nullptr;
   const bool wide = a.N >= 4096;
   const int prof = PROF_GEMV;
+#define WDR_SK_T(...) __VA_ARGS__
+#define WDR_SK(T, G, B, LDS)                                                                      \
+  do {                                                                                            \
+    if (a.b_packed) wdr_launch(prof, bytes, flops, k_skinny<EPI, WDR_SK_T T, true>, G, B, LDS, s, a); \
+    else wdr_launch(prof, bytes, flops, k_skinny<EPI, WDR_SK_T T, false>, G, B, LDS, s, a);       \
+  } while (0)
   if (!wide) {
     if (a.K > 2048) {
       WDR_CHECK(!ln, "row projection: LN prologue needs K <= 1280");
       if (mt >= 4 && rows_pair_tiles()) {
         const int m2 = std::min(mt, rows_mt_max());
         const dim3 g2(cdiv(a.N, 16), cdiv(mt, m2));
-        if (m2 >= 4) wdr_launch(prof, bytes, flops, k_skinny<EPI, 4, 1, 16, false, 2>, g2, dim3(1024), 0, s, a);
-        else if (m2 == 3) wdr_launch(prof, bytes, flops, k_skinny<EPI, 3, 1, 16, false, 5>, g2, dim3(1024), 0, s, a);
-        else wdr_launch(prof, bytes, flops, k_skinny<EPI, 2, 1, 16, false, 5>, g2, dim3(1024), 0, s, a);
+        if (m2 >= 4) WDR_SK((4, 1, 16, false, 2), g2, dim3(1024), 0);
+        else if (m2 == 3) WDR_SK((3, 1, 16, false, 5), g2, dim3(1024), 0);
+        else WDR_SK((2, 1, 16, false, 5), g2, dim3(1024), 0);
         return;
       }
-      wdr_launch(prof, bytes, flops, k_skinny<EPI, 1, 1, 16, false, 12>, dim3(cdiv(a.N, 16), mt), dim3(1024), 0, s, a);
+      WDR_SK((1, 1, 16, false, 12), dim3(cdiv(a.N, 16), mt), dim3(1024), 0);
       return;
     }
     if (!ln && mt > 2 && rows_pair_tiles()) {
       const int m2 = std::min(mt, rows_mt_max());
       const dim3 g2(cdiv(a.N, 16), cdiv(mt, m2));
-      if (m2 >= 5) wdr_launch(prof, bytes, flops, k_skinny<EPI, 5, 1, 8>, g2, dim3(512), 0, s, a);
-      else if (m2 == 4) wdr_launch(prof, bytes, flops, k_skinny<EPI, 4, 1, 8>, g2, dim3(512), 0, s, a);
-      else if (m2 == 3) wdr_launch(prof, bytes, flops, k_skinny<EPI, 3, 1, 8>, g2, dim3(512), 0, s, a);
-      else wdr_launch(prof, bytes, flops, k_skinny<EPI, 2, 1, 8>, g2, dim3(512), 0, s, a);
+      if (m2 >= 5) WDR_SK((5, 1, 8, false, 0), g2, dim3(512), 0);
+      else if (m2 == 4) WDR_SK((4, 1, 8, false, 0), g2, dim3(512), 0);
+      else if (m2 == 3) WDR_SK((3, 1, 8, false, 0), g2, dim3(512), 0);
+      else WDR_SK((2, 1, 8, false, 0), g2, dim3(512), 0);
       return;
     }
     dim3 grid(cdiv(a.N, 16), mt), blk(512);
-    if (ln) wdr_launch(prof, bytes, flops, k_skinny<EPI, 1, 1, 8, true>, grid, blk, skinny_ln_lds<EPI, 1, 1, 8>(a.K), s, a);
-    else wdr_launch(prof, bytes, flops, k_skinny<EPI, 1, 1, 8>, grid, blk, 0, s, a);
+    if (ln) WDR_SK((1, 1, 8, true, 0), grid, blk, (skinny_ln_lds<EPI, 1, 1, 8>(a.K)));
+    else WDR_SK((1, 1, 8, false, 0), grid, blk, 0);
     return;
   }
   const int mtw = std::min(mt, ln ? 2 : 4);
   dim3 grid(cdiv(a.N, 32), cdiv(mt, mtw)), blk(512);
 #define WDR_RW(MTV)                                                                                        \
-  if (ln) wdr_launch(prof, bytes, flops, k_skinny<EPI, MTV, 2, 8, true>, grid, blk, skinny_ln_lds<EPI, MTV, 2, 8>(a.K), s, a); \
-  else wdr_launch(prof, bytes, flops, k_skinny<EPI, MTV, 2, 8>, grid, blk, 0, s, a);
+  if (ln) WDR_SK((MTV, 2, 8, true, 0), grid, blk, (skinny_ln_lds<EPI, MTV, 2, 8>(a.K)));                   \
+  else WDR_SK((MTV, 2, 8, false, 0), grid, blk, 0);
   if (mtw == 1) { WDR_RW(1) }
   else if (mtw == 2) { WDR_RW(2) }
   else if (mtw == 3) { WDR_RW(3) }
   else { WDR_RW(4) }
 #undef WDR_RW
+#undef WDR_SK
+#undef WDR_SK_T
+}
+
+__global__ __launch_bounds__(256) void k_pack_rows(const f16* w, f16* out, int N, int K, long long chunks) {
+  const long long c = (long long)blockIdx.x * 256 + threadIdx.x;
+  if (c >= chunks) return;
+  const int kt = K >> 5;
+  const long long tile = c >> 6;
+  const int l = (int)(c & 63);
+  const int n = (int)(tile / kt) * 16 + (l & 15), k = (int)(tile % kt) * 32 + (l >> 4) * 8;
+  f16x8 v = {};
+  if (n < N) v = *(const f16x8*)(w + (size_t)n * K + k);
+  *(f16x8*)(out + c * 8) = v;
+}
+
+size_t packed_rows_elems(int N, int K) { return (size_t)cdiv(N, 16) * 16 * K; }
+
+void launch_pack_rows(const f16* w, f16* out, int N, int K, hipStream_t s) {
+  WDR_CHECK(N >= 1 && K >= 32 && K % 32 == 0 && w != out, "pack rows: K % 32, out of place");
+  const long long chunks = (long long)packed_rows_elems(N, K) / 8;
+  WDR_KLAUNCH(k_pack_rows, dim3((unsigned)((chunks + 255) / 256)), dim3(256), 0, s, w, out, N, K, chunks);
+  WDR_HIP(hipGetLastError());
 }
 
 static void launch_rows(const ProjArgs& a, hipStream_t s) {
   WDR_CHECK(a.K % 32 == 0 && a.lda % 8 == 0 && a.ldb % 8 == 0, "row projection: K % 32, lda / ldb % 8");
+  WDR_CHECK(!a.b_packed || a.ldb == a.K, "row projection: packed weights have no row stride (ldb == K)");
   WDR_CHECK(!a.ln_x || (a.K <= 1280 && a.K % 128 == 0), "row projection LN prologue: K <= 1280, K % 128 == 0");
   WDR_CHECK(a.epi != EPI_QKV_CACHE || (a.kc && a.vc && a.row_seq && a.row_pos && a.d > 0), "qkv-cache epilogue args");
   switch (a.epi) {
@@ -1568,6 +1603,7 @@
     launch_rows(a, s);
     return;
   }
+  WDR_CHECK(!a.b_packed, "projection: only the row kernel reads fragment-order weights");
   WDR_CHECK(a.K % 8 == 0 && a.lda % 8 == 0 && a.ldb % 8 == 0, "projection: K/lda/ldb must be multiples of 8");
   WDR_CHECK(a.N % GB_N == 0, "gemm: N must be a multiple of 128");
   WDR_CHECK(a.K % GB_K == 0, "gemm: K must be a multiple of 32");
diff --git a/whisper-diarize-rs_amd/csrc/rows.cpp b/whisper-diarize-rs_amd/csrc/rows.cpp
--- a/whisper-diarize-rs_amd/csrc/rows.cpp
+++ b/whisper-diarize-rs_amd/csrc/rows.cpp
@@ -165,10 +165,11 @@
   static const int ln_env = getenv("WDR_ROWS_LN_FUSE") ? atoi(getenv("WDR_ROWS_LN_FUSE")) : -1;
   const int fuse_qkv = ln_env >= 0 ? ln_env : 48, fuse_xq = ln_env >= 0 ? ln_env : 64,
             fuse_fc1 = ln_env >= 0 ? ln_env : 24, fuse_logits = ln_env >= 0 ? ln_env : 0;
-  auto P = [&](const f16* A, int lda, const f16* W, const float* b, void* out, int ldo, int N, int K, int epi,
-               const float* lng = nullptr, const float* lnb = nullptr, int fuse_max = 0) {
+  auto P = [&](const f16* A, int lda, const f16* W, unsigned pk, const float* b, void* out, int ldo, int N, int K,
+               int epi, const float* lng = nullptr, const float* lnb = nullptr, int fuse_max = 0) {
     ProjArgs a{A, lda, W, K, b, out, ldo, nullptr, 0, R, N, K, epi};
     a.rows_mma = 1;
+    a.b_packed = (md.rows_packed & pk) ? 1 : 0;
     if (lng) {
       if (R <= fuse_max) {
         a.ln_x = io.xd;
@@ -190,7 +191,7 @@
     const DecLayer& e = md.dec[l];
     f16* kc = io.kc + (size_t)l * io.layer_stride;
     f16* vc = io.vc + (size_t)l * io.layer_stride;
-    ProjArgs q = P(nullptr, d, e.w_qkv, e.b_qkv, io.qkvd, 3 * d, 3 * d, d, EPI_QKV_CACHE, e.ln1_g, e.ln1_b, fuse_qkv);
+    ProjArgs q = P(nullptr, d, e.w_qkv, Model::PK_QKV, e.b_qkv, io.qkvd, 3 * d, 3 * d, d, EPI_QKV_CACHE, e.ln1_g, e.ln1_b, fuse_qkv);
     q.kc = kc;
     q.vc = vc;
     q.seq_stride = io.seq_stride;
@@ -200,8 +201,8 @@
     launch_proj(q, s);
     DecSelfArgs sa{io.qkvd, 3 * d, kc, vc, io.seq_stride, d, io.seq, io.pos, io.attd, d, scale};
     launch_dec_self_attn(sa, R, H, s);
-    launch_proj(P(io.attd, d, e.w_o, e.b_o, io.xd, d, d, d, EPI_F32_RESID), s);
-    launch_proj(P(nullptr, d, e.w_xq, e.b_xq, io.qx, d, d, d, EPI_F16, e.ln2_g, e.ln2_b, fuse_xq), s);
+    launch_proj(P(io.attd, d, e.w_o, Model::PK_O, e.b_o, io.xd, d, d, d, EPI_F32_RESID), s);
+    launch_proj(P(nullptr, d, e.w_xq, Model::PK_XQ, e.b_xq, io.qx, d, d, d, EPI_F16, e.ln2_g, e.ln2_b, fuse_xq), s);
     XAttnArgs xa{io.qx, d, nullptr, nullptr, 64, XKV_T, R, H, scale, io.part_o, io.part_ml, io.attd, d};
     xa.row_k = io.xkv;
     xa.layer_off = xkv_k_off(l, H);
@@ -227,13 +228,16 @@
     }
     if (ctx.aheads_per_layer.size() == (size_t)L) cap_slot0 += (int)ctx.aheads_per_layer[l].size();
     if (l + 1 >= l_stop) return;
-    launch_proj(P(io.attd, d, e.w_xo, e.b_xo, io.xd, d, d, d, EPI_F32_RESID), s);
-    launch_proj(P(nullptr, d, e.w_fc1, e.b_fc1, io.mlpd, 4 * d, 4 * d, d, EPI_F16_GELU, e.ln3_g, e.ln3_b, fuse_fc1), s);
-    launch_proj(P(io.mlpd, 4 * d, e.w_fc2, e.b_fc2, io.xd, d, d, 4 * d, EPI_F32_RESID), s);
+    launch_proj(P(io.attd, d, e.w_xo, Model::PK_XO, e.b_xo, io.xd, d, d, d, EPI_F32_RESID), s);
+    launch_proj(P(nullptr, d, e.w_fc1, Model::PK_FC1, e.b_fc1, io.mlpd, 4 * d, 4 * d, d, EPI_F16_GELU, e.ln3_g, e.ln3_b, fuse_fc1), s);
+    launch_proj(P(io.mlpd, 4 * d, e.w_fc2, Model::PK_FC2, e.b_fc2, io.xd, d, d, 4 * d, EPI_F32_RESID), s);
   }
   if (io.n_logit > 0) {
-    ProjArgs a{nullptr, d, md.tok_emb, d, nullptr, io.logits, io.ldlogits, nullptr, 0, io.n_logit, hp.n_vocab, d, EPI_F32};
+    const bool pk = (md.rows_packed & Model::PK_LOGITS) != 0;
+    ProjArgs a{nullptr, d, pk ? md.tok_emb_pk : md.tok_emb, d, nullptr, io.logits, io.ldlogits, nullptr, 0, io.n_logit,
+               hp.n_vocab, d, EPI_F32};
     a.rows_mma = 1;
+    a.b_packed = pk ? 1 : 0;
     if (io.n_logit <= fuse_logits) {
       a.ln_x = io.xd;
       a.ldln = d;
diff --git a/whisper-diarize-rs_amd/csrc/whisper.h b/whisper-diarize-rs_amd/csrc/whisper.h
--- a/whisper-diarize-rs_amd/csrc/whisper.h
+++ b/whisper-diarize-rs_amd/csrc/whisper.h
@@ -61,6 +61,10 @@
   f16* w_xkv = nullptr;
   float* b_xkv = nullptr;
   f16* tok_emb = nullptr;
+  enum { PK_QKV = 1, PK_O = 2, PK_XQ = 4, PK_XO = 8, PK_FC1 = 16, PK_FC2 = 32, PK_LOGITS = 64 };
+  unsigned rows_packed = 0;
+  f16* tok_emb_pk = nullptr;
+  DevMem tok_emb_pk_mem;
   float *dec_pos = nullptr, *ln_g = nullptr, *ln_b = nullptr;
   float *mel_filters = nullptr, *hann = nullptr, *cos_tab = nullptr, *sin_tab = nullptr;
   DevMem storage;
diff --git a/whisper-diarize-rs_amd/csrc/whisper_ctx.cpp b/whisper-diarize-rs_amd/csrc/whisper_ctx.cpp
--- a/whisper-diarize-rs_amd/csrc/whisper_ctx.cpp
+++ b/whisper-diarize-rs_amd/csrc/whisper_ctx.cpp
@@ -538,8 +538,34 @@
     aheads_dev = DevMem(std::max<size_t>(4, flat.size() * 4));
     if (!flat.empty()) WDR_HIP(wdr_memcpy_async(aheads_dev.p, flat.data(), flat.size() * 4, hipMemcpyHostToDevice, s));
   }
+  DevMem pscratch;
+  {
+    const char* pe = getenv("WDR_ROWS_PACKED");
+    m.rows_packed = pe ? (unsigned)strtoul(pe, nullptr, 0) & 0x7f : 0x7fu;
+    if (m.rows_packed & 0x3f) pscratch = DevMem((size_t)4 * dt * dt * 2);
+    auto pack = [&](f16* w, int N, int K) {
+      launch_pack_rows(w, pscratch.as<f16>(), N, K, s);
+      WDR_HIP(wdr_memcpy_async(w, pscratch.p, (size_t)N * K * 2, hipMemcpyDeviceToDevice, s));
+    };
+    for (int i = 0; i < L; ++i) {
+      const DecLayer& e = m.dec[i];
+      if (m.rows_packed & Model::PK_QKV) pack(e.w_qkv, 3 * dt, dt);
+      if (m.rows_packed & Model::PK_O) pack(e.w_o, dt, dt);
+      if (m.rows_packed & Model::PK_XQ) pack(e.w_xq, dt, dt);
+      if (m.rows_packed & Model::PK_XO) pack(e.w_xo, dt, dt);
+      if (m.rows_packed & Model::PK_FC1) pack(e.w_fc1, 4 * dt, dt);
+      if (m.rows_packed & Model::PK_FC2) pack(e.w_fc2, dt, 4 * dt);
+    }
+    if (m.rows_packed & Model::PK_LOGITS) {
+      m.tok_emb_pk_mem = DevMem(packed_rows_elems(hp.n_vocab, dt) * 2);
+      m.tok_emb_pk = m.tok_emb_pk_mem.as<f16>();
+      m.weight_bytes += m.tok_emb_pk_mem.bytes;
+      launch_pack_rows(m.tok_emb, m.tok_emb_pk, hp.n_vocab, dt, s);
+    }
+  }
   WDR_HIP(hipStreamSynchronize(s));
   qstage = DevMem();
+  pscratch = DevMem();
   {
     const char* e = getenv("WDR_DECODE_CHAINS");
     max_chains = std::max(1, std::min(64, e ? atoi(e) : 40));
diff --git a/whisper-diarize-rs_amd/wdr/__init__.py b/whisper-diarize-rs_amd/wdr/__init__.py
--- a/whisper-diarize-rs_amd/wdr/__init__.py
+++ b/whisper-diarize-rs_amd/wdr/__init__.py
@@ -666,7 +666,7 @@
     return out
 
 
-def dbg_proj_qkv(a, w, bias, row_seq, row_pos, kc, vc):
+def dbg_proj_qkv(a, w, bias, row_seq, row_pos, kc, vc, packed=False):
     ab, wb = _h16(a), _h16(w)
     M, K = ab.shape
     d = wb.shape[0] // 3
@@ -677,10 +677,10 @@
         raise ValueError("dbg_proj_qkv: a [M][K], w [3 d][K], kc / vc [n_seq][T][d], row_seq / row_pos [M]")
     b = None if bias is None else np.ascontiguousarray(bias, np.float32)
     q = np.zeros((M, d), np.float32)
-    L.check(L.load().wdr_dbg_proj_qkv(ab.ctypes.data_as(_U16P), wb.ctypes.data_as(_U16P),
-                                      None if b is None else b.ctypes.data_as(_F32P), M, d, K,
-                                      rs.ctypes.data_as(_I32P), rp.ctypes.data_as(_I32P), n_seq, T,
-                                      kb.ctypes.data_as(_U16P), vb.ctypes.data_as(_U16P), q.ctypes.data_as(_F32P)))
+    fn = L.load().wdr_dbg_proj_qkv_packed if packed else L.load().wdr_dbg_proj_qkv
+    L.check(fn(ab.ctypes.data_as(_U16P), wb.ctypes.data_as(_U16P), None if b is None else b.ctypes.data_as(_F32P), M, d, K,
+               rs.ctypes.data_as(_I32P), rp.ctypes.data_as(_I32P), n_seq, T, kb.ctypes.data_as(_U16P),
+               vb.ctypes.data_as(_U16P), q.ctypes.data_as(_F32P)))
     return q, kb.view(np.float16), vb.view(np.float16)
 
 
diff --git a/whisper-diarize-rs_amd/wdr/_lib.py b/whisper-diarize-rs_amd/wdr/_lib.py
--- a/whisper-diarize-rs_amd/wdr/_lib.py
+++ b/whisper-diarize-rs_amd/wdr/_lib.py
@@ -193,6 +193,9 @@
                                     P(f32)]),
     "wdr_dbg_proj_qkv": (C.c_int, [P(C.c_uint16), P(C.c_uint16), P(f32), i32, i32, i32, P(i32), P(i32), i32, i32,
                                    P(C.c_uint16), P(C.c_uint16), P(f32)]),
+    "wdr_dbg_proj_qkv_packed": (C.c_int, [P(C.c_uint16), P(C.c_uint16), P(f32), i32, i32, i32, P(i32), P(i32), i32,
+                                          i32, P(C.c_uint16), P(C.c_uint16), P(f32)]),
+    "wdr_dbg_pack_rows": (C.c_int, [P(C.c_uint16), i32, i32, P(C.c_uint16)]),
     "wdr_dbg_logits_topk": (C.c_int, [vp, P(f32), i32, P(i32), P(f32), f32, i32, i32, P(i32), P(f32)]),
     "wdr_dbg_logits_probs": (C.c_int, [vp, P(f32), i32, P(i32), P(f32), f32, i32, P(f32), P(f32)]),
     "wdr_dbg_kv_rows": (C.c_int, [vp, i32, i32, i32, P(C.c_uint16), P(C.c_uint16)]),
```

After: 907.3 (median of 6 runs). 1.04x the previous value.
